# talmolab/track-mjx

Hardware: AMD Instinct MI355X
Metric: env-steps/sec (whole node), rodent task @ 4096 envs/GPU (higher is better)
Workload: dtype f32

## Files before the change

include/tmjx.h:

```cpp
#ifndef TMJX_H
#define TMJX_H
#include <stddef.h>
#include <stdint.h>

#ifdef __cplusplus
extern "C" {
#endif

#define TMJX_OK 0
#define TMJX_EINVAL (-22)
#define TMJX_ENOMEM (-12)
#define TMJX_EHIP (-5)

typedef struct tmjx_model tmjx_model;

typedef struct tmjx_layout_t {
  int32_t nq, nv, nu, nbody, ncon, nefc, obs_size, ref_obs_size, n_metrics, window;
  int32_t qpos, qvel, act, qacc_warmstart, time;
  int32_t xpos, xmat_torso, qfrc_actuator;
  int32_t prev_ctrl, action_buffer, done, steps_f;
  int32_t first_phys, first_obs, first_prev_ctrl;
  int32_t state_rows;
  int32_t i_clip_idx, i_start_frame, i_buffer_index, i_nan_count, istate_rows;
  int32_t ws_rows;
// ... 42 lines not shown
int tmjx_gae(const float *truncation, const float *termination, const float *rewards, const float *values,
             const float *bootstrap, float lambda_, float discount, float *vs, float *advantages, int T, int B,
             void *stream);

typedef struct {
  int32_t T, B, A, Z;
  float reward_scaling, discounting, gae_lambda, clip_eps, entropy_cost, kl_weight;
  int32_t normalize_advantage;
  int32_t accumulate;
} tmjx_ppo_cfg_t;
int tmjx_ppo_scratch_floats(int T, int B);
int tmjx_ppo_loss(const tmjx_ppo_cfg_t *cfg, const float *logits, const float *raw_action, const float *behaviour_logp,
                  const float *noise, const float *baseline, const float *bootstrap, const float *reward, const float *discount,
                  const float *truncation, const float *fc2, float *dlogits, float *dbaseline, float *dfc2, float *scratch,
                  float *out, void *stream);

#define TMJX_PPO_PHASE_A 1
#define TMJX_PPO_PHASE_B 2
#define TMJX_PPO_PHASE_C 4
#define TMJX_PPO_PHASE_D 8
int tmjx_ppo_loss_phases(const tmjx_ppo_cfg_t *cfg, const float *logits, const float *raw_action, const float *behaviour_logp,
                         const float *noise, const float *baseline, const float *bootstrap, const float *reward, const float *discount,
                         const float *truncation, const float *fc2, float *dlogits, float *dbaseline, float *dfc2, float *scratch,
                         float *out, int phases, void *stream);

int tmjx_silu_ln_partial_floats(int rows, int H);
int tmjx_silu_ln_fwd(const float *z, const float *bias, const float *gamma, const float *beta, float *y, float *stats, int rows, int H,
                     float eps, void *stream);
int tmjx_silu_ln_bwd(const float *dy, const float *z, const float *bias, const float *gamma, const float *stats, float *dz, float *grads,
                     float *partial, int rows, int H, void *stream);
int tmjx_silu_ln_fwd_bf16(const float *z, const float *bias, const float *gamma, const float *beta, uint16_t *y16, int ldy16, float *stats, int rows, int H,
                          float eps, void *stream);
int tmjx_silu_ln_bwd_bf16(const float *dy, const float *z, const float *bias, const float *gamma, const float *stats, uint16_t *dz16, int lddz16, float *grads,
                          float *partial, int rows, int H, void *stream);

int tmjx_gather_normalize(const float *src, const int64_t *idx, const float *mean, const float *std, float *out, int T, int R, int B,
                          int W, void *stream);
int tmjx_gather_minibatch(const float *obs, const float *next_last, const float *raw_action, const float *log_prob, const float *reward, const float *discount,
                          const float *truncation, const int64_t *idx, const float *mean, const float *std, float *obs_n, float *next_n, float *raw_action_g,
                          float *scalars_g, int T, int R, int B, int W, int A, void *stream);
#define TMJX_MINIBATCH_STATE_WORDS (16 + 16 * 64)
typedef struct tmjx_minibatch_t {
  const float *obs, *next_last, *raw_action, *log_prob, *reward, *discount, *truncation;
  const int64_t *perm;
  const float *mean, *std;
  float *obs_n, *next_n, *raw_action_g, *scalars_g;
  float *eps, *noise;
  int64_t *state;
  uint64_t seed;
  int32_t T, R, B, W, A, Z, advance;
} tmjx_minibatch_t;
int tmjx_minibatch_begin(const tmjx_minibatch_t *mb, void *stream);
int tmjx_minibatch_begin_bf16(const tmjx_minibatch_t *mb, uint16_t *obs_n16, int ld16, void *stream);
int tmjx_philox4x32_10(const uint32_t *ctr_key_dev, uint32_t *out_dev, void *stream);

int tmjx_latent_concat_bwd(const float *dx, const float *eps, const float *fc2, float *dfc2, int n, int Z, int dx_stride, void *stream);
int tmjx_latent_concat_bwd_add(const float *dx, const float *eps, const float *fc2, const float *add, float *dfc2, int n, int Z, int dx_stride,
                               void *stream);

int tmjx_latent_concat(const float *fc2, const float *eps, const float *obs, float *x, int n, int Z, int obs_w, int ref_w,
                       int64_t obs_s0, int64_t obs_s1, const float *mean, const float *std, int x_stride, uint64_t seed, const int64_t *rng_state,
                       void *stream);
int tmjx_sample_action(const float *logits, const float *noise, float *raw, float *action_t, float *logp, int n, int A, uint64_t seed,
                       int64_t *rng_state, void *stream);

int tmjx_linear_act_ok(const float *A, int64_t lda, const float *W, int ldw, int K);
int tmjx_linear_act(const float *A, int64_t lda, const float *W, int ldw, const float *bias, float *C, int M, int N, int K,
                    const float *mean, const float *inv_std, void *stream);
int tmjx_linear_nolds(const float *A, int64_t sa_row, int64_t sa_k, const float *W, const float *bias, float *C, int M, int N, int K,
                      void *stream);
int tmjx_linear_nolds_norm(const float *A, int64_t sa_row, int64_t sa_k, const float *W, const float *bias, float *C, int M, int N, int K,
                           const float *mean, const float *inv_std, void *stream);

int tmjx_linear_nolds_bf16(const float *A, int64_t sa_row, int64_t sa_k, const uint16_t *W, int ldw, const float *bias, float *C, int M, int N, int K,
                           const float *mean, const float *inv_std, void *stream);

int tmjx_colsum_scratch_floats(int width);
int tmjx_colsum(const float *src, float *out, float *scratch, int rows, int width, void *stream);

typedef struct tmjx_colsum_problem_t { const float *partial; float *out; int32_t rows, width; } tmjx_colsum_problem_t;
int tmjx_colsum_grouped(const tmjx_colsum_problem_t *problems, int n, void *stream);

int tmjx_adam_clip(float *param, const float *grad, float *exp_avg, float *exp_avg_sq, const float *grad_norm, long long n, float lr,
                   float beta1, float beta2, float eps, float bias_correction1, float bias_correction2, float max_norm, void *stream);
int tmjx_adam_norm_floats(void);
int tmjx_adam_clip_norm(float *param, const float *grad, float *exp_avg, float *exp_avg_sq, float *norm_scratch, float *norm_out, long long n, float lr,
                        float beta1, float beta2, float eps, float bias_correction1, float bias_correction2, float max_norm, void *stream);
int tmjx_adam_clip_norm_frozen(float *param, const float *grad, float *exp_avg, float *exp_avg_sq, float *norm_scratch, float *norm_out, long long n,
                               long long frozen_lo, long long frozen_hi, float lr, float beta1, float beta2, float eps, float bias_correction1,
                               float bias_correction2, float max_norm, void *stream);

int tmjx_gemm_nt(const float *A, int lda, const float *W, int ldw, const float *bias, float *C, int ldc, int M, int N, int K, void *stream);
int tmjx_gemm_nn(const float *A, int lda, const float *W, int ldw, float *C, int ldc, int M, int N, int K, void *stream);
int tmjx_gemm_nt_silu_ln_ok(const float *A, int lda, const float *W, int ldw, int N);
int tmjx_gemm_nt_silu_ln(const float *A, int lda, const float *W, int ldw, const float *bias, const float *gamma, const float *beta, float *Z, float *Y,
                         int ldc, float *stats, int M, int N, int K, float eps, void *stream);
int tmjx_gemm_nn_ln_bwd_ok(const float *dY, int ldy, const float *W, int ldw, int N);
long long tmjx_gemm_nn_ln_bwd_partial_floats(int M, int N);
int tmjx_gemm_nn_ln_bwd(const float *dY, int ldy, const float *W, int ldw, const float *z, const float *bias, const float *gamma, const float *stats,
                        float *dz, float *partial, int M, int N, int K, void *stream);
int tmjx_gemm_nt_silu_ok(const float *A, int lda, const float *W, int ldw);
int tmjx_gemm_nt_silu(const float *A, int lda, const float *W, int ldw, const float *bias, float *Z, float *Y, int ldc, int M, int N, int K, void *stream);
int tmjx_silu_fwd(const float *z, const float *bias, float *y, long long rows, int N, void *stream);
int tmjx_silu_bwd(const float *dy, const float *z, const float *bias, float *dz, long long rows, int N, void *stream);
int tmjx_gemm_nn_silu_bwd_ok(const float *dY, int ldy, const float *W, int ldw);
int tmjx_gemm_nn_silu_bwd(const float *dY, int ldy, const float *W, int ldw, const float *z, const float *bias, float *dZ, int M, int N, int K, void *stream);
int tmjx_silu_bwd_rank1(const float *dy1, const float *w1, const float *z, const float *bias, float *dz, long long rows, int N, void *stream);
long long tmjx_head_dw_scratch_floats(int M, int K);
int tmjx_head_dw(const float *dy1, const float *x, int ldx, float *dw, float *db, float *scratch, int M, int K, void *stream);
#define TMJX_CHAIN_MAX_HIDDEN 4
typedef struct { const float *W, *bias, *gamma, *beta; float *z, *y, *stats; int32_t K, ldw; } tmjx_chain_layer_t;
typedef struct {
  const float *A; int32_t lda, M, n_hidden, epi;
  tmjx_chain_layer_t hidden[TMJX_CHAIN_MAX_HIDDEN];
  const float *Wf, *bf; float *outf; int32_t Nf, ldwf, ldof;
  float eps;
  int32_t rows_alloc;
  void *prof;
} tmjx_chain_fwd_t;
int tmjx_chain_rows(int M);
int tmjx_chain_fwd_ok(const tmjx_chain_fwd_t *chain);
int tmjx_chain_fwd(const tmjx_chain_fwd_t *chain, void *stream);
typedef struct { const float *W; int32_t ldw; const float *z, *bias, *gamma, *stats; float *dz, *partial; } tmjx_chain_bwd_stage_t;
typedef struct {
  const float *G; int32_t ldg, Kg, M, n_stages, epi;
  tmjx_chain_bwd_stage_t stage[TMJX_CHAIN_MAX_HIDDEN];
  const float *W0; int32_t ldw0, dx_cols; float *dx; int32_t lddx;
  int32_t rows_alloc;
  void *prof;
} tmjx_chain_bwd_t;
int tmjx_chain_bwd_ok(const tmjx_chain_bwd_t *chain);
int tmjx_chain_bwd(const tmjx_chain_bwd_t *chain, void *stream);

int tmjx_head_fwd_ok(const float *x, int ldx, const float *w, int K);
int tmjx_head_fwd(const float *x, int ldx, const float *w, const float *bias, float *y, int M, int K, void *stream);
long long tmjx_gemm_dw_scratch_floats(int M, int N, int K);
int tmjx_gemm_dw(const float *dY, int ldy, const float *X, int ldx, float *dW, float *db, float *scratch, int M, int N, int K, void *stream);
typedef struct tmjx_dw_problem_t {
  const float *dY, *X;
  float *dW, *db, *scratch;
  int32_t ldy, ldx, lddw, M, N, K;
} tmjx_dw_problem_t;
int tmjx_gemm_dw_grouped(const tmjx_dw_problem_t *problems, int n, void *stream);

typedef struct tmjx_bf16_shadow_t {
  const float *src;
  uint16_t *dst, *dst_t;
  int32_t N, K, ld_src, ld_dst, ld_dst_t;
} tmjx_bf16_shadow_t;
int tmjx_bf16_shadow(const tmjx_bf16_shadow_t *items, int n, void *stream);
int tmjx_bgemm_nt(const void *A, int a_is_f32, int lda, const uint16_t *B, int ldb, const float *bias, float *C, int ldc, int M, int N, int K,
                  void *stream);
int tmjx_bgemm_row_tile_ok(int N);
int tmjx_bf16_z_bytes(void);
long long tmjx_bgemm_partial_floats(int M, int N, int sums);
int tmjx_bgemm_ln_fwd(const void *A, int a_is_f32, int lda, const uint16_t *B, int ldb, const float *bias, const float *gamma, const float *beta, uint16_t *Z16, int ldz,
                      uint16_t *Y16, int ldy16, float *stats, int M, int N, int K, float eps, void *stream);
int tmjx_bgemm_ln_bwd(const void *dY, int dy_is_f32, int ldy, const uint16_t *Bt, int ldb, const uint16_t *z16, int ldz, const float *bias, const float *gamma,
                      const float *stats, uint16_t *dZ16, int lddz, float *partial, int M, int N, int K, void *stream);
int tmjx_bgemm_silu_fwd(const void *A, int a_is_f32, int lda, const uint16_t *B, int ldb, const float *bias, uint16_t *Z16, int ldz, uint16_t *Y16, int ldy16,
                        float *Yf, int ldyf, int M, int N, int K, void *stream);
int tmjx_bgemm_silu_bwd(const void *dY, int dy_is_f32, int ldy, const uint16_t *Bt, int ldb, const uint16_t *z16, int ldz, const float *bias, uint16_t *dZ16, int lddz,
                        float *partial, int M, int N, int K, void *stream);
int tmjx_bf_silu_bwd(const float *dY, int ldy, const uint16_t *z16, int ldz, const float *bias, uint16_t *dZ16, int lddz, float *partial, int M, int N, void *stream);
int tmjx_bf_silu_bwd_rank1(const float *dy1, const float *w1, const uint16_t *z16, int ldz, const float *bias, uint16_t *dZ16, int lddz, float *partial, int M, int N,
                           void *stream);
long long tmjx_bgemm_dw_scratch_floats(int M, int N, int K);
int tmjx_bgemm_dw(const void *dY, int y_is_f32, int ldy, const void *X, int x_is_f32, int ldx, float *dW, int lddw, float *db, float *scratch,
                  int M, int N, int K, void *stream);
typedef struct tmjx_bdw_problem_t {
  const void *dY, *X;
  float *dW, *db, *scratch;
  int32_t y_is_f32, x_is_f32, ldy, ldx, lddw, M, N, K;
} tmjx_bdw_problem_t;
int tmjx_bgemm_dw_grouped(const tmjx_bdw_problem_t *problems, int n, int target_wgs, void *stream);

typedef struct tmjx_rollout_store_t {
  const float *obs; float *obs_dst0, *obs_dst1;
  const float *raw; float *raw_dst;
  const float *logp; float *logp_dst;
  const float *reward; float *reward_dst;
  const float *done; float *discount_dst;
  const float *trunc; float *trunc_dst;
  int32_t n, W, A;
  float *obs_dst2;
} tmjx_rollout_store_t;
int tmjx_rollout_store(const tmjx_rollout_store_t *s, void *stream);
int tmjx_clips_upload_velocities(tmjx_model *m, const float *velocity, const float *joints_velocity, int n_clips, int n_frames);
int tmjx_clips_share(tmjx_model *m, const tmjx_model *owner);

int tmjx_stats_scratch_floats(int W);
int tmjx_stats_sums(const float *src, const float *mean, float *sums, float *scratch, long long rows, int W, void *stream);
int tmjx_stats_apply(const float *sums, float n_added, float *count, float *mean, float *summed_variance, float *std, int W, float std_min,
                     float std_max, void *stream);
int tmjx_stats_apply_pinned(const float *sums, float n_added, float *count, float *mean, float *summed_variance, float *std, int W, int pin_lo,
                            float std_min, float std_max, void *stream);
// ... 299 lines not shown
```

track_mjx_amd/agent/losses.py:

```python
from __future__ import annotations

import ctypes as C

import torch

from .. import hip as _hip
from .networks import NormalTanh


def compute_gae(truncation, termination, rewards, values, bootstrap_value, lambda_: float = 1.0, discount: float = 0.99):
    T, B = rewards.shape
    args = [x.detach().contiguous().float() for x in (truncation, termination, rewards, values, bootstrap_value)]
    if not args[0].is_cuda:
        raise _hip.TmjxError("compute_gae runs on the GPU only (tmjx_gae); there is no CPU fallback")
    vs = torch.empty((T, B), dtype=torch.float32, device=rewards.device)
    adv = torch.empty_like(vs)
    L = _hip.lib()
    with torch.cuda.device(rewards.device):
        stream = C.c_void_p(torch.cuda.current_stream(rewards.device).cuda_stream)
        _hip.check(L.tmjx_gae(*[C.c_void_p(a.data_ptr()) for a in args], float(lambda_), float(discount),
                              C.c_void_p(vs.data_ptr()), C.c_void_p(adv.data_ptr()), T, B, stream), "tmjx_gae")
    return vs, adv


def gather_normalize(src: torch.Tensor, idx: torch.Tensor, normalizer) -> torch.Tensor:
    squeeze = src.dim() == 2
    if squeeze:
        src = src.unsqueeze(0)
    T, R, W = src.shape
    out = torch.empty((T, idx.shape[0], W), dtype=torch.float32, device=src.device)
    L = _hip.lib()
    with torch.cuda.device(src.device):
        stream = C.c_void_p(torch.cuda.current_stream(src.device).cuda_stream)
        _hip.check(L.tmjx_gather_normalize(*[C.c_void_p(t.data_ptr()) for t in (src, idx, normalizer.mean, normalizer.std, out)], T, R,
                                           idx.shape[0], W, stream), "tmjx_gather_normalize")
    return out[0] if squeeze else out


def gather_minibatch(buf: dict, idx: torch.Tensor, normalizer) -> dict:
    obs, nxt, act = buf["observation"], buf["next_observation_last"], buf["raw_action"]
    T, R, W = obs.shape
    B, A = idx.shape[0], act.shape[-1]
    f32 = dict(dtype=torch.float32, device=obs.device)
    obs_n, next_n = torch.empty((T, B, W), **f32), torch.empty((B, W), **f32)
    act_g, sc = torch.empty((T, B, A), **f32), torch.empty((4, T, B), **f32)
    p = lambda t: C.c_void_p(t.data_ptr())
    with torch.cuda.device(obs.device):
        _hip.check(_hip.lib().tmjx_gather_minibatch(p(obs), p(nxt), p(act), p(buf["log_prob"]), p(buf["reward"]), p(buf["discount"]), p(buf["truncation"]), p(idx),
                                                    p(normalizer.mean), p(normalizer.std), p(obs_n), p(next_n), p(act_g), p(sc), T, R, B, W, A,
                                                    C.c_void_p(torch.cuda.current_stream(obs.device).cuda_stream)), "tmjx_gather_minibatch")
    return {"observation_normalized": obs_n, "next_observation_last_normalized": next_n, "raw_action": act_g, "log_prob": sc[0], "reward": sc[1],
            "discount": sc[2], "truncation": sc[3]}


def minibatch_begin(buf: dict, perm: torch.Tensor, state: torch.Tensor, seed: int, normalizer, latents: int, advance: bool = True,
                    obs16: torch.Tensor | None = None) -> dict:
    obs, nxt, act = buf["observation"], buf["next_observation_last"], buf["raw_action"]
    T, R, W = obs.shape
    B, A = int(buf["_B"]), act.shape[-1]
    f32 = dict(dtype=torch.float32, device=obs.device)
    obs_n, next_n = torch.empty((T, B, W), **f32), torch.empty((B, W), **f32)
    act_g, sc = torch.empty((T, B, A), **f32), torch.empty((4, T, B), **f32)
    eps, noise = torch.empty((T, B, latents), **f32), torch.empty((T, B, A), **f32)
    d = lambda t: t.data_ptr()
    m = _hip.Minibatch(d(obs), d(nxt), d(act), d(buf["log_prob"]), d(buf["reward"]), d(buf["discount"]), d(buf["truncation"]), d(perm), d(normalizer.mean),
                       d(normalizer.std), d(obs_n), d(next_n), d(act_g), d(sc), d(eps), d(noise), d(state), seed & (2 ** 64 - 1), T, R, B, W, A, latents, int(advance))
    out = {"observation_normalized": obs_n, "next_observation_last_normalized": next_n, "raw_action": act_g, "log_prob": sc[0], "reward": sc[1],
           "discount": sc[2], "truncation": sc[3], "latent_eps": eps, "entropy_noise": noise}
    with torch.cuda.device(obs.device):
        stream = C.c_void_p(torch.cuda.current_stream(obs.device).cuda_stream)
        if obs16 is not None:
            assert obs16.dtype == torch.bfloat16 and obs16.shape[0] == T * B and obs16.shape[1] >= W and obs16.is_contiguous()
            _hip.check(_hip.lib().tmjx_minibatch_begin_bf16(C.byref(m), C.c_void_p(obs16.data_ptr()), obs16.shape[1], stream), "tmjx_minibatch_begin_bf16")
            out["observation_normalized_bf16"] = obs16
        else:
            _hip.check(_hip.lib().tmjx_minibatch_begin(C.byref(m), stream), "tmjx_minibatch_begin")
    return out


def create_ramp_schedule(max_value: float = 0.1, min_value: float = 0.0001, ramp_steps: int = 1000, warmup_steps: int = 0):
    def schedule_fn(step: float) -> float:
        if step < warmup_steps:
            return min_value
        progress = min(max((step - warmup_steps) / ramp_steps, min_value), 1.0)
        return progress * max_value
    return schedule_fn


class _FusedLossHead(torch.autograd.Function):

    @staticmethod
    def forward(ctx, logits, baseline, fc2, raw_action, behaviour_logp, noise, bootstrap, reward, discount, truncation, cfg):
        T, B = reward.shape
        dev = logits.device
        args = [a.detach().contiguous().float() for a in (logits, raw_action, behaviour_logp, noise, baseline, bootstrap, reward,
                                                          discount, truncation, fc2)]
        dlogits, dbaseline, dfc2 = torch.empty_like(args[0]), torch.empty_like(args[4]), torch.empty_like(args[9])
        L = _hip.lib()
        scratch = torch.empty(L.tmjx_ppo_scratch_floats(T, B), dtype=torch.float32, device=dev)
        out = torch.empty(8, dtype=torch.float32, device=dev)
        c = _hip.PpoCfg(T, B, raw_action.shape[-1], fc2.shape[-1] // 2, cfg["reward_scaling"], cfg["discounting"], cfg["gae_lambda"],
                        cfg["clipping_epsilon"], cfg["entropy_cost"], cfg["kl_weight"], int(cfg["normalize_advantage"]), 0)
        with torch.cuda.device(dev):
            stream = C.c_void_p(torch.cuda.current_stream(dev).cuda_stream)
            ptr = [C.c_void_p(a.data_ptr()) for a in args + [dlogits, dbaseline, dfc2, scratch, out]]
            _hip.check(L.tmjx_ppo_loss(C.byref(c), *ptr, stream), "tmjx_ppo_loss")
        ctx.save_for_backward(dlogits, dbaseline, dfc2)
        ctx.mark_non_differentiable(out)
        return out[0].clone(), out

    @staticmethod
    def backward(ctx, g_total, _g_out):
        dlogits, dbaseline, dfc2 = ctx.saved_tensors
        return (dlogits * g_total, dbaseline * g_total, dfc2 * g_total) + (None,) * 8


def ppo_loss_and_output_grads(policy, value, normalizer, data: dict, *, entropy_cost: float = 1e-4, kl_weight: float = 1e-3,
                              discounting: float = 0.9, reward_scaling: float = 1.0, gae_lambda: float = 0.95,
                              clipping_epsilon: float = 0.3, normalize_advantage: bool = True, side_stream=None, acc_out: torch.Tensor | None = None,
                              scalars_on_side: bool = False):
    obs = data["observation_normalized"] if "observation_normalized" in data else normalizer.normalize(data["observation"])
    nxt = data["next_observation_last_normalized"] if "next_observation_last_normalized" in data else normalizer.normalize(data["next_observation_last"])
    T, B = data["reward"].shape
    dev = obs.device
    L = _hip.lib()
    phased = side_stream is not None and T <= 24
    cfg_of = lambda A_, Z_: _hip.PpoCfg(T, B, A_, Z_, reward_scaling, discounting, gae_lambda, clipping_epsilon, entropy_cost, kl_weight,
                                        int(normalize_advantage), int(acc_out is not None))
    f32 = lambda a: a.detach().contiguous().float()
    if side_stream is not None:
        cur = torch.cuda.current_stream(dev)
        with torch.no_grad():
            scratch = torch.empty(L.tmjx_ppo_scratch_floats(T, B), dtype=torch.float32, device=dev)
            out = torch.empty(8, dtype=torch.float32, device=dev) if acc_out is None else acc_out
            row = [f32(data[k]) for k in ("raw_action", "log_prob", "reward", "discount", "truncation")]
        side_stream.wait_stream(cur)
        with torch.cuda.stream(side_stream):
            with torch.no_grad():
                bootstrap = value(nxt)
            baseline = value(obs)
            if phased:
                with torch.no_grad():
                    bl, bs = f32(baseline), f32(bootstrap)
        logits, fc2 = policy(obs, eps=data.get("latent_eps"), return_fc2=True)
        if not phased:
            cur.wait_stream(side_stream)
        baseline.record_stream(cur); bootstrap.record_stream(cur)
    else:
        logits, fc2 = policy(obs, eps=data.get("latent_eps"), return_fc2=True)
        baseline = value(obs)
        with torch.no_grad():
            bootstrap = value(nxt)
    with torch.no_grad():
        noise = data["entropy_noise"] if "entropy_noise" in data else torch.randn(data["raw_action"].shape, dtype=torch.float32, device=logits.device)
        if phased:
            lg, nz, f2 = f32(logits), f32(noise), f32(fc2)
            dlogits, dbaseline, dfc2 = torch.empty_like(lg), torch.empty_like(bl), torch.empty_like(f2)
            c = cfg_of(data["raw_action"].shape[-1], fc2.shape[-1] // 2)
            args = [lg, row[0], row[1], nz, bl, bs, row[2], row[3], row[4], f2]
            ptr = [C.c_void_p(a.data_ptr()) for a in args + [dlogits, dbaseline, dfc2, scratch, out]]
            for t_ in (scratch, out, dbaseline, *row):
                t_.record_stream(side_stream)
            for t_ in (bl, bs):
                t_.record_stream(cur)

            def phase(mask, stream):
                _hip.check(L.tmjx_ppo_loss_phases(C.byref(c), *ptr, mask, C.c_void_p(stream.cuda_stream)), "tmjx_ppo_loss_phases")
            with torch.cuda.device(dev):
                phase(2, side_stream)
                cur.wait_stream(side_stream)
                phase(1 | 4, cur)
                if scalars_on_side:
                    side_stream.wait_stream(cur)
                    phase(8, side_stream)
                else:
                    phase(8, cur)
            args9 = f2
        else:
            args = [f32(a) for a in (logits, data["raw_action"], data["log_prob"], noise, baseline, bootstrap, data["reward"],
                                     data["discount"], data["truncation"], fc2)]
            dlogits, dbaseline, dfc2 = torch.empty_like(args[0]), torch.empty_like(args[4]), torch.empty_like(args[9])
            if side_stream is None:
                scratch = torch.empty(L.tmjx_ppo_scratch_floats(T, B), dtype=torch.float32, device=dev)
                out = torch.empty(8, dtype=torch.float32, device=dev) if acc_out is None else acc_out
            c = cfg_of(data["raw_action"].shape[-1], fc2.shape[-1] // 2)
            with torch.cuda.device(dev):
                stream = C.c_void_p(torch.cuda.current_stream(dev).cuda_stream)
                ptr = [C.c_void_p(a.data_ptr()) for a in args + [dlogits, dbaseline, dfc2, scratch, out]]
                _hip.check(L.tmjx_ppo_loss(C.byref(c), *ptr, stream), "tmjx_ppo_loss")
            args9 = args[9]
    metrics = {"total_loss": out[0], "policy_loss": out[1], "v_loss": out[2], "kl_latent_loss": out[4], "entropy_loss": out[3]}
    handle = getattr(policy, "latent_grad_handle", None)
    if handle is not None and handle.matches(fc2) and args9.data_ptr() == fc2.data_ptr():
        handle.add(dfc2.view(-1, fc2.shape[-1]))
        return metrics, (logits, baseline), (dlogits.view_as(logits), dbaseline.view_as(baseline)), out
    return metrics, (logits, baseline, fc2), (dlogits.view_as(logits), dbaseline.view_as(baseline), dfc2.view_as(fc2)), out


def compute_ppo_loss_fused(policy, value, normalizer, data: dict, *, entropy_cost: float = 1e-4, kl_weight: float = 1e-3,
                           discounting: float = 0.9, reward_scaling: float = 1.0, gae_lambda: float = 0.95,
                           clipping_epsilon: float = 0.3, normalize_advantage: bool = True):
    obs = data["observation_normalized"] if "observation_normalized" in data else normalizer.normalize(data["observation"])
# ... 54 lines not shown
```

track_mjx_amd/agent/networks.py:

```python
from __future__ import annotations

import math
import os
from typing import Sequence

import torch
import torch.nn as nn
import torch.nn.functional as F


def _lecun_uniform_(w: torch.Tensor) -> None:
    fan_in = w.shape[1]
    lim = math.sqrt(3.0 / fan_in)
    with torch.no_grad():
        w.uniform_(-lim, lim)


def _lecun_normal_(w: torch.Tensor) -> None:
    fan_in = w.shape[1]
    std = math.sqrt(1.0 / fan_in) / 0.87962566103423978
    with torch.no_grad():
        nn.init.trunc_normal_(w, mean=0.0, std=std, a=-2 * std, b=2 * std)


# ... 172 lines not shown
    return dz[:, :N], partial.view(-1, N)


class Bf16Shadows:

    def __init__(self, linears, need_t=None):
        from .. import hip as _hip
        self.lins = list(linears)
        need_t = set(self.lins if need_t is None else need_t)
        dev = self.lins[0].weight.device
        self.w, self.wt = {}, {}
        items = []
        for lin in self.lins:
            N, K = lin.weight.shape
            self.w[lin] = torch.zeros((N, _ceil64(K)), dtype=torch.bfloat16, device=dev)
            if lin in need_t:
                self.wt[lin] = torch.zeros((K, _ceil64(N)), dtype=torch.bfloat16, device=dev)
            t = self.wt.get(lin)
            items.append(_hip.Bf16Shadow(lin.weight.data_ptr(), self.w[lin].data_ptr(), t.data_ptr() if t is not None else None, N, K, lin.weight.stride(0),
                                         self.w[lin].stride(0), t.stride(0) if t is not None else 0))
        self._chunks = [(_hip.Bf16Shadow * len(items[i:i + 24]))(*items[i:i + 24]) for i in range(0, len(items), 24)]
        self._ptrs = [lin.weight.data_ptr() for lin in self.lins]

    def refresh(self) -> None:
        if self._ptrs != [lin.weight.data_ptr() for lin in self.lins]:
            raise RuntimeError("a parameter moved after its bf16 shadow was built (build the shadows after the flat optimiser re-seats the parameters)")
        dev = self.lins[0].weight.device
        for arr in self._chunks:
            _launch("tmjx_bf16_shadow", dev, arr, len(arr))


def _bf16_ok(x, lin) -> bool:
    sh = gemm_inputs.shadows
    return (gemm_inputs.dtype == torch.bfloat16 and sh is not None and lin in sh.w and x.is_cuda and x.dtype == torch.float32
            and lin.out_features % 4 == 0)


def _colsum(dy: torch.Tensor) -> torch.Tensor:
    if not (dy.is_cuda and dy.dtype == torch.float32 and dy.dim() == 2 and dy.is_contiguous() and dy.shape[0] >= 1024):
        return dy.sum(0)
    from .. import hip as _hip
    rows, width = dy.shape
    out = torch.empty(width, dtype=torch.float32, device=dy.device)
    scratch = torch.empty(_hip.lib().tmjx_colsum_scratch_floats(width), dtype=torch.float32, device=dy.device)
    _launch("tmjx_colsum", dy.device, _p(dy), _p(out), _p(scratch), rows, width)
    return out


class deferred_weight_grads:
    active = None

    def __enter__(self):
        self.problems, self.keep, self.colsums = [], [], []
        self.bproblems = []
        self.seen: set = set()
        deferred_weight_grads.active = self
        return self

    def __exit__(self, *a):
        deferred_weight_grads.active = None
        return False

    @staticmethod
    def _aligned(t):
        return t.data_ptr() % 16 == 0 and t.stride(0) % 4 == 0 and t.stride(1) == 1

    def try_add(self, dy2, x2, w, b):
        gw, gb = w.grad, (b.grad if b is not None else None)
        if gw is None or (b is not None and gb is None) or len(self.problems) >= 16:
            return None
        if not (self._aligned(dy2) and self._aligned(x2) and gw.stride(1) == 1 and gw.shape == w.shape):
            return None
        if id(w) in self.seen:
            mine = [q for q in self.problems if q[2].data_ptr() == gw.data_ptr()]
            self.problems = [q for q in self.problems if q[2].data_ptr() != gw.data_ptr()]
            self._launch_problems(mine)
            return None
        self.seen.add(id(w))
        self.problems.append((dy2, x2, gw, gb))
        return gw, gb

    def launch(self):
        from .. import hip as _hip
        if self.colsums:
            dev = self.colsums[0][0].device
            arr = (_hip.ColsumProblem * len(self.colsums))(*[_hip.ColsumProblem(pt.data_ptr(), g.data_ptr(), nb, wd) for pt, g, nb, wd in self.colsums])
            _launch("tmjx_colsum_grouped", dev, arr, len(self.colsums))
            self.keep += [t for c in self.colsums for t in c[:2]]
            self.colsums = []
        self._launch_problems(self.problems)
        self.problems = []
        self._launch_bproblems()

    def _launch_bproblems(self):
        from .. import hip as _hip
        probs, self.bproblems = self.bproblems, []
        if not probs:
            return
        L = _hip.lib()
        dev = probs[0][0].device
        for at in range(0, len(probs), 24):
            grp = probs[at:at + 24]
            sizes = [int(L.tmjx_bgemm_dw_scratch_floats(dy.shape[0], dy.shape[1], x.shape[1])) for dy, x, _, _ in grp]
            scratch = torch.empty(sum((n + 3) // 4 * 4 for n in sizes), dtype=torch.float32, device=dev)
            arr = (_hip.BdwProblem * len(grp))()
            off = 0
            for i, (dy, x, dw, db) in enumerate(grp):
                N, K = dy.shape[1], x.shape[1]
                arr[i] = _hip.BdwProblem(dy.data_ptr(), x.data_ptr(), dw.data_ptr(), db.data_ptr() if db is not None else None, scratch.data_ptr() + 4 * off,
                                         int(dy.dtype == torch.float32), int(x.dtype == torch.float32), _ld(dy), _ld(x), dw.stride(0) if N > 1 else max(dw.stride(0), K),
                                         dy.shape[0], N, K)
                off += (sizes[i] + 3) // 4 * 4
            _launch("tmjx_bgemm_dw_grouped", dev, arr, len(grp), 0)
            self.keep += [scratch] + [t for q in grp for t in q[:2]]

    def _launch_problems(self, problems):
        from .. import hip as _hip
        if not problems:
            return
        L = _hip.lib()
        dev = problems[0][0].device
        sizes = [int(L.tmjx_gemm_dw_scratch_floats(dy.shape[0], dy.shape[1], x.shape[1])) for dy, x, _, _ in problems]
        scratch = torch.empty(sum((n + 3) // 4 * 4 for n in sizes), dtype=torch.float32, device=dev)
        arr = (_hip.DwProblem * len(problems))()
        off = 0
        for i, (dy, x, gw, gb) in enumerate(problems):
            arr[i] = _hip.DwProblem(dy.data_ptr(), x.data_ptr(), gw.data_ptr(), gb.data_ptr() if gb is not None else None,
                                    scratch.data_ptr() + 4 * off, dy.stride(0), x.stride(0), gw.stride(0), dy.shape[0], dy.shape[1], x.shape[1])
            off += (sizes[i] + 3) // 4 * 4
        _launch("tmjx_gemm_dw_grouped", dev, arr, len(problems))
        self.keep += [scratch] + [t for q in problems for t in q[:2]]


def chain_fwd_desc(x2, hidden, final=None, kind="ln", eps=1e-6, out=None):
    from .. import hip as _hip
    M, dev = x2.shape[0], x2.device
    d = _hip.ChainFwd()
    d.A, d.lda, d.M, d.n_hidden, d.epi, d.eps = x2.data_ptr(), x2.stride(0), M, len(hidden), 1 if kind == "ln" else 3, float(eps)
    saved = []
    d.rows_alloc = rows = int(_hip.lib().tmjx_chain_rows(M))
    for l, h in enumerate(hidden):
        w, b = h[0], h[1]
        z = torch.empty((M, 256), dtype=torch.float32, device=dev)
        y = torch.empty((rows, 256), dtype=torch.float32, device=dev)[:M]
        st = torch.empty((M, 2), dtype=torch.float32, device=dev) if kind == "ln" else None
        L = d.hidden[l]
        L.W, L.bias, L.z, L.y, L.K, L.ldw = w.data_ptr(), b.data_ptr(), z.data_ptr(), y.data_ptr(), w.shape[1], w.stride(0)
        if kind == "ln":
            L.gamma, L.beta, L.stats = h[2].data_ptr(), h[3].data_ptr(), st.data_ptr()
        saved.append((z, y, st))
    if final is not None:
        wf, bf = final
        Nf = wf.shape[0]
        if out is None:
            out = torch.empty((M,) if Nf == 1 else (M, Nf), dtype=torch.float32, device=dev)
        d.Wf, d.bf, d.outf, d.Nf, d.ldwf, d.ldof = wf.data_ptr(), (bf.data_ptr() if bf is not None else None), out.data_ptr(), Nf, wf.stride(0), (1 if Nf == 1 else out.stride(0))
    return d, saved, out


def chain_fwd(x2, hidden, final=None, kind="ln", eps=1e-6):
    import ctypes as C
    d, saved, out = chain_fwd_desc(x2, hidden, final, kind, eps)
    _launch("tmjx_chain_fwd", x2.device, C.byref(d))
    return saved, out


def chain_fwd_ok(x2, hidden, final=None, kind="ln") -> bool:
    import ctypes as C
    from .. import hip as _hip
    if os.environ.get("TMJX_NO_CHAIN") or not (x2.is_cuda and x2.dtype == torch.float32 and x2.dim() == 2 and x2.stride(1) == 1):
        return False
    if any(h[0].shape[0] != 256 for h in hidden) or not (1 <= len(hidden) <= 4):
        return False
    return bool(_hip.lib().tmjx_chain_fwd_ok(C.byref(chain_fwd_desc(x2[:1], hidden, final, kind)[0])))


def chain_bwd(g, final_w, blocks, kind="ln", w0=None, dx_cols=None, prof=None, dx_ld=None):
    import ctypes as C
    from .. import hip as _hip
    L = _hip.lib()
    M, dev = g.shape[0], g.device
    d = _hip.ChainBwd()
    head = g.dim() == 1
# ... 182 lines not shown
        for L in layers:
            out += [grads.get(id(p)) for p in L.params()]
        return (dx, None, None, None, None, *out)


def bf16_chain(x, layers, dx_cols=None, last_y_f32=False):
    params = [p for L in layers for p in L.params()]
    return _BfChainFn.apply(x, layers, gemm_inputs.shadows, dx_cols, last_y_f32, *params)


def _bf16_chain_ok(x) -> bool:
    sh = gemm_inputs.shadows
    return gemm_inputs.dtype == torch.bfloat16 and sh is not None and x.is_cuda and x.dtype in (torch.float32, torch.bfloat16)



class _F32ChainFn(torch.autograd.Function):

    @staticmethod
    def forward(ctx, x, layers, dx_cols, *params):
        x2 = _rows2d(x)
        hid, last = layers[:-1], layers[-1]
        kind = hid[0].kind
        hidden = [(L.lin.weight, L.lin.bias, L.norm.weight, L.norm.bias) if kind == "ln" else (L.lin.weight, L.lin.bias) for L in hid]
        eps = float(hid[0].norm.eps) if kind == "ln" else 0.0
        saved, out = chain_fwd(x2, hidden, (last.lin.weight, last.lin.bias), kind, eps)
        flat = [t for z, y, st in saved for t in ((z, y, st) if kind == "ln" else (z, y))]
        ctx.save_for_backward(x2, *flat, *params)
        ctx.layers, ctx.dx_cols, ctx.x_shape, ctx.kind, ctx.nflat = layers, dx_cols, x.shape, kind, len(flat)
        return out.view(*x.shape[:-1], last.lin.out_features) if last.kind == "dense" else out.view(*x.shape[:-1], 1)

    @staticmethod
    def backward(ctx, dout):
        from .. import hip as _hip
        layers, kind = ctx.layers, ctx.kind
        hid, last = layers[:-1], layers[-1]
        st_ = ctx.saved_tensors
        x2, flat, params = st_[0], st_[1:1 + ctx.nflat], st_[1 + ctx.nflat:]
        per = 3 if kind == "ln" else 2
        saved = [flat[per * i:per * i + per] for i in range(len(hid))]
        pit = iter(params)
        P = [[next(pit) for _ in L.params()] for L in layers]
        Lh = _hip.lib()
        dev = dout.device
        M = x2.shape[0]
        d = deferred_weight_grads.active
        grads: dict = {}
        wf, bf = P[-1][0], P[-1][1]
        y_last = saved[-1][1]
        if last.kind == "head":
            g = dout.reshape(-1)
            g = g if g.is_contiguous() else g.contiguous()
            K = wf.shape[1]
            dwh, dbh = torch.empty((1, K), dtype=torch.float32, device=dev), torch.empty(1, dtype=torch.float32, device=dev)
            scratch = torch.empty(int(Lh.tmjx_head_dw_scratch_floats(M, K)), dtype=torch.float32, device=dev)
            _launch("tmjx_head_dw", dev, _p(g), _p(y_last), y_last.stride(0), _p(dwh), _p(dbh), _p(scratch), M, K)
            grads[(len(layers) - 1, 0)], grads[(len(layers) - 1, 1)] = dwh, dbh
            ctx._keep = scratch
        else:
            g = _rows2d(dout)
            if g.data_ptr() % 16 or g.stride(0) % 4:
                g = g.contiguous()
            got = d.try_add(g, y_last, last.lin.weight, last.lin.bias) if d is not None else None
            dw, db = got if got is not None else gemm_dw(g, y_last, True)
            grads[(len(layers) - 1, 0)], grads[(len(layers) - 1, 1)] = dw, db
        if kind == "ln":
            blocks = [(P[l][0], saved[l][0], P[l][1], P[l][2], saved[l][2]) for l in range(len(hid) - 1, -1, -1)]
        else:
            blocks = [(P[l][0], saved[l][0], P[l][1]) for l in range(len(hid) - 1, -1, -1)]
        want_dx = ctx.needs_input_grad[0]
        cols = (x2.shape[1] if ctx.dx_cols is None else int(ctx.dx_cols)) if want_dx else None
        dzs, partials, dx = chain_bwd(g, wf, blocks, kind, P[0][0] if want_dx else None, cols, dx_ld=x2.shape[1] if want_dx else None)
        for i, dz in enumerate(dzs):
            l = len(hid) - 1 - i
            L = hid[l]
            xin = x2 if l == 0 else saved[l - 1][1]
            if kind == "ln":
                got = d.try_add(dz, xin, L.lin.weight, None) if d is not None else None
                grads[(l, 0)] = got[0] if got is not None else gemm_dw(dz, xin, False)[0]
                g3 = torch.empty((3, 256), dtype=torch.float32, device=dev)
                nblk = partials[i].numel() // 768
                if d is not None and len(d.colsums) < 16:
                    d.colsums.append((partials[i], g3, nblk, 768))
                else:
                    one = (_hip.ColsumProblem * 1)(_hip.ColsumProblem(partials[i].data_ptr(), g3.data_ptr(), nblk, 768))
                    _launch("tmjx_colsum_grouped", dev, one, 1)
                grads[(l, 2)], grads[(l, 3)], grads[(l, 1)] = g3[0], g3[1], g3[2]
            else:
                got = d.try_add(dz, xin, L.lin.weight, L.lin.bias) if d is not None else None
                grads[(l, 0)], grads[(l, 1)] = got if got is not None else gemm_dw(dz, xin, True)
        out = [grads.get((l, j)) for l, L in enumerate(layers) for j in range(len(L.params()))]
        return (dx.view(ctx.x_shape) if dx is not None else None, None, None, *out)


def f32_chain(x, layers, dx_cols=None):
    params = [p for L in layers for p in L.params()]
    return _F32ChainFn.apply(x, layers, dx_cols, *params)


def _f32_chain_ok(x, layers, dx_cols=None) -> bool:
    if gemm_inputs.dtype is not None or torch.is_autocast_enabled() or os.environ.get("TMJX_NO_CHAIN") or not (x.is_cuda and x.dtype == torch.float32):
        return False
    if x.requires_grad and torch.is_grad_enabled() and (x.shape[-1] if dx_cols is None else int(dx_cols)) > 128:
        return False
    hid, last = layers[:-1], layers[-1]
    if not hid or any(L.lin.out_features != 256 or L.lin.bias is None for L in hid) or last.lin.bias is None or last.lin.in_features != 256:
        return False
    kind = hid[0].kind
    hidden = [(L.lin.weight, L.lin.bias, L.norm.weight, L.norm.bias) if kind == "ln" else (L.lin.weight, L.lin.bias) for L in hid]
    return chain_fwd_ok(_rows2d(x), hidden, (last.lin.weight, last.lin.bias), kind)


class _BlockLink:
    __slots__ = ("y_ptr", "y_shape", "ctx", "dz_given", "grads")

    def __init__(self):
        self.y_ptr, self.y_shape, self.ctx, self.dz_given, self.grads = None, None, None, False, None


class ln_bwd_links:
    active = False
    last = None

    def __enter__(self):
        self._prev = (ln_bwd_links.active, ln_bwd_links.last)
        ln_bwd_links.active, ln_bwd_links.last = not os.environ.get("TMJX_NO_LN_BWD_FUSION"), None
        return self

    def __exit__(self, *a):
        ln_bwd_links.active, ln_bwd_links.last = self._prev
        return False

    @staticmethod
    def producer_of(x2):
# ... 310 lines not shown
        d = deferred_weight_grads.active
        got = d.try_add(dz, x2, ctx.param, None) if d is not None else None
        dw = got[0] if got is not None else gemm_dw(dz, x2, False)[0]
        return dx, dw, grads[2], grads[0], grads[1], None, None


class _Block(nn.Module):
    FUSED_WIDTHS = (64, 128, 256, 512, 1024)

    def __init__(self, i: int, o: int):
        super().__init__()
        self.dense = _dense(i, o)
        self.norm = nn.LayerNorm(o, eps=1e-6)
        self.dx_cols = None

    def forward(self, x):
        if x.is_cuda and x.dtype == torch.float32 and self.dense.out_features in self.FUSED_WIDTHS and not torch.is_autocast_enabled():
            x2 = _rows2d(x)
            if torch.is_grad_enabled() and _block_fusable(x2, self.dense.weight):
                y = _HipBlockFn.apply(x2, self.dense.weight, self.dense.bias, self.norm.weight, self.norm.bias, self.norm.eps, self.dx_cols)
                return y.view(*x.shape[:-1], self.dense.out_features)
            if _bf16_ok(x2, self.dense):
                if torch.is_grad_enabled():
                    z = _BfDenseFn.apply(x2, self.dense.weight, None, self.dense, self.dx_cols)
                else:
                    z = bgemm_nt(x2, gemm_inputs.shadows.w[self.dense], self.dense.out_features, self.dense.in_features)
            elif not torch.is_grad_enabled():
                z = gemm_nt(x2, self.dense.weight)
            else:
                z = _HipDenseFn.apply(x2, self.dense.weight, None, self.dx_cols)
            y = _SiluLayerNormFn.apply(z, self.dense.bias, self.norm.weight, self.norm.bias, self.norm.eps)
            return y.view(*x.shape[:-1], self.dense.out_features)
        return self.norm(F.silu(self.dense(x)))


class _LatentConcatFn(torch.autograd.Function):

    @staticmethod
    def forward(ctx, fc2, eps, obs, ref, handle=None):
        ctx.handle = handle
        n, Z = eps.shape
        W = obs.shape[1]
        fc2, eps, obs = fc2.contiguous(), eps.contiguous(), obs.contiguous()
        wd = Z + W - ref
        x = torch.empty((n, (wd + 3) // 4 * 4), dtype=torch.float32, device=fc2.device)
        _launch("tmjx_latent_concat", fc2.device, _p(fc2), _p(eps), _p(obs), _p(x), n, Z, W, ref, obs.stride(0), obs.stride(1), None, None, x.shape[1], 0, None)
        ctx.save_for_backward(fc2, eps)
        return x[:, :wd]

    @staticmethod
    def backward(ctx, dx):
        fc2, eps = ctx.saved_tensors
        n, Z = eps.shape
        dx = dx.contiguous()
        dfc2 = torch.empty_like(fc2)
        add = ctx.handle.take() if ctx.handle is not None else None
        if add is not None and (add.shape != fc2.shape or not add.is_contiguous()):
            raise RuntimeError("_LatentConcatFn: the pending fc2 gradient does not fit this forward pass")
        if add is None:
            _launch("tmjx_latent_concat_bwd", fc2.device, _p(dx), _p(eps), _p(fc2), _p(dfc2), n, Z, dx.shape[1])
        else:
            _launch("tmjx_latent_concat_bwd_add", fc2.device, _p(dx), _p(eps), _p(fc2), _p(add), _p(dfc2), n, Z, dx.shape[1])
        return dfc2, None, None, None, None


class LatentGradHandle:

    def __init__(self, fc2: torch.Tensor):
        self.ptr, self.shape, self._g = fc2.data_ptr(), tuple(fc2.shape), None

    def matches(self, fc2: torch.Tensor) -> bool:
        return fc2.data_ptr() == self.ptr

    def add(self, g: torch.Tensor) -> None:
        if self._g is not None:
            raise RuntimeError("LatentGradHandle: a gradient is already parked on this forward pass")
        self._g = g

    def take(self):
        g, self._g = self._g, None
        return g

    @property
    def pending(self) -> bool:
        return self._g is not None


class IntentionPolicy(nn.Module):

    def __init__(self, obs_size: int, reference_obs_size: int, action_size: int, latents: int = 60,
                 encoder_layers: Sequence[int] = (1024, 1024), decoder_layers: Sequence[int] = (1024, 1024)):
        super().__init__()
        self.reference_obs_size, self.latents, self.action_size = reference_obs_size, latents, action_size
        enc, d = [], reference_obs_size
        for h in encoder_layers:
            enc.append(_Block(d, h)); d = h
        self.encoder = nn.Sequential(*enc)
        self.fc2 = _dense(d, 2 * latents, _lecun_normal_)
        dec, d = [], latents + (obs_size - reference_obs_size)
        for h in decoder_layers:
            dec.append(_Block(d, h)); d = h
        self.decoder = nn.Sequential(*dec)
        dec[0].dx_cols = latents
        self.head = _dense(d, 2 * action_size)

    def forward(self, obs: torch.Tensor, eps: torch.Tensor | None = None, deterministic: bool = False, return_fc2: bool = False):
        traj = obs[..., :self.reference_obs_size]
        prev, self.latent_grad_handle = getattr(self, "latent_grad_handle", None), None
        if prev is not None and prev.pending:
            raise RuntimeError("IntentionPolicy: the fc2 gradient parked on the previous forward pass (LatentGradHandle.add) was never consumed by a "
                               "backward pass through that forward — it would have been dropped")
        chains = _bf16_chain_ok(obs) and all(m.out_features % 4 == 0 for m in (self.fc2, self.head))
        if chains:
            if getattr(self, "_enc_chain", None) is None:
                self._enc_chain = [_Layer("ln", b.dense, b.norm) for b in self.encoder] + [_Layer("dense", self.fc2)]
                self._dec_chain = [_Layer("ln", b.dense, b.norm) for b in self.decoder] + [_Layer("dense", self.head)]
            fc2 = bf16_chain(traj, self._enc_chain)
        else:
            if getattr(self, "_enc_f32", None) is None and obs.is_cuda:
                self._enc_f32 = [_Layer("ln", b.dense, b.norm) for b in self.encoder] + [_Layer("dense", self.fc2)]
                self._dec_f32 = [_Layer("ln", b.dense, b.norm) for b in self.decoder] + [_Layer("dense", self.head)]
            if obs.is_cuda and _f32_chain_ok(traj, self._enc_f32):
                fc2 = f32_chain(traj, self._enc_f32)
            else:
                with ln_bwd_links():
                    h = self.encoder(traj)
                    fc2 = self.fc2(h)
        mean, logvar = torch.chunk(fc2, 2, dim=-1)
        if (not deterministic and fc2.is_cuda and fc2.dtype == torch.float32 and obs.dtype == torch.float32 and not torch.is_autocast_enabled()
                and fc2.numel() >= 2 * self.latents * 1024):
            lead = fc2.shape[:-1]
            if eps is None:
                eps = torch.randn_like(mean)
            handle = LatentGradHandle(fc2.reshape(-1, fc2.shape[-1])) if (fc2.requires_grad and fc2.is_contiguous()) else None
            x = _LatentConcatFn.apply(fc2.reshape(-1, fc2.shape[-1]), eps.reshape(-1, self.latents), obs.reshape(-1, obs.shape[-1]), self.reference_obs_size, handle)
            self.latent_grad_handle = handle
            x = x.view(*lead, x.shape[-1])
            if chains:
                logits = bf16_chain(x, self._dec_chain, dx_cols=self.latents)
            elif _f32_chain_ok(x, self._dec_f32, self.latents):
                logits = f32_chain(x, self._dec_f32, dx_cols=self.latents)
            else:
                with ln_bwd_links():
                    logits = self.head(self.decoder(x))
            if return_fc2:
                return logits, fc2
            return logits, mean, logvar
        if deterministic:
            z = mean
        else:
            if eps is None:
                eps = torch.randn_like(mean)
            z = mean + eps * torch.exp(0.5 * logvar)
        x = torch.cat([z, obs[..., self.reference_obs_size:]], dim=-1)
        logits = bf16_chain(x, self._dec_chain) if chains else self.head(self.decoder(x))
        if return_fc2:
            return logits, fc2
        return logits, mean, logvar


class DecoderNet(nn.Module):

    def __init__(self, input_size: int, action_size: int, decoder_layers: Sequence[int] = (1024, 1024)):
        super().__init__()
        self.action_size = action_size
        dec, d = [], input_size
        for h in decoder_layers:
            dec.append(_Block(d, h)); d = h
        self.decoder = nn.Sequential(*dec)
        self.head = _dense(d, 2 * action_size)

    def forward(self, x: torch.Tensor) -> torch.Tensor:
        return self.head(self.decoder(x))


class _NoCtx:
    def save_for_backward(self, *a):
        pass


class ValueNet(nn.Module):

    def __init__(self, obs_size: int, hidden: Sequence[int] = (1024, 1024)):
        super().__init__()
        layers, d = [], obs_size
        for h in hidden:
            layers += [_dense(d, h), nn.SiLU()]; d = h
        layers.append(_dense(d, 1))
# ... 139 lines not shown
```

track_mjx_amd/agent/ppo.py:

```python
from __future__ import annotations

import logging
import math
import time
from typing import Callable

import numpy as np
import torch
import torch.distributed as dist

from . import losses as _losses
from .networks import Bf16Shadows, IntentionPolicy, NormalTanh, RunningStatistics, ValueNet, deferred_weight_grads, gemm_inputs


import contextlib
import gc
import os


@contextlib.contextmanager
def _capture(graph):
    gc.collect()
    enabled = gc.isenabled()
    gc.disable()
# ... 559 lines not shown
        offs = [0]
        for e in self.envs:
            offs.append(offs[-1] + e.num_envs)
        self._refresh_padded_weights()
        cur = torch.cuda.current_stream(self.dev) if self._streams else None
        if self._streams:
            for sg in self._streams:
                sg.wait_stream(cur)
        jax_noise = self.sgd_keys is not None and self.act_rng == "jax"
        if jax_noise:
            self.sgd_keys.start_unrolls()
        for u in range(self.unrolls):
            if jax_noise:
                self.sgd_keys.start_unroll()
            for t in range(T):
                if jax_noise:
                    eps_np, noise_np = self.sgd_keys.act_noise(n_local, self.policy.latents, self.policy.action_size)
                    eps_all, noise_all = torch.from_numpy(eps_np).to(self.dev), torch.from_numpy(noise_np).to(self.dev)
                    if self._streams:
                        ev = torch.cuda.Event()
                        ev.record(torch.cuda.current_stream(self.dev))
                        for sg in self._streams:
                            sg.wait_event(ev)
                            eps_all.record_stream(sg); noise_all.record_stream(sg)
                for g, env in enumerate(self.envs):
                    sl = slice(u * n_local + offs[g], u * n_local + offs[g + 1])
                    with torch.cuda.stream(self._streams[g]) if self._streams else _nullctx():
                        st = self.states[g]
                        if u == 0 and t == 0:
                            self.buf["observation"][0, sl] = st.obs
                            if self._obs_rm is not None:
                                self._obs_rm[g].copy_(st.obs)
                        if jax_noise:
                            action, extra = self.act(st.obs, draws=(eps_all[offs[g]:offs[g + 1]], noise_all[offs[g]:offs[g + 1]]))
                        else:
                            action, extra = self._act_graphed(st.obs if self._obs_rm is None else self._obs_rm[g], g)
                        st = env.step(st, action)
                        nxt = self.buf["observation"][t + 1, sl] if t + 1 < T else self.buf["next_observation_last"][sl]
                        nxt1 = self.buf["observation"][0, slice(sl.start + n_local, sl.stop + n_local)] if (t + 1 == T and u + 1 < self.unrolls) else None
                        self._store_transition(env, st, extra, nxt, nxt1, t, sl, None if self._obs_rm is None else self._obs_rm[g])
                        self.states[g] = st
        if self._streams:
            for sg in self._streams:
                cur.wait_stream(sg)

    def _self_advancing(self) -> bool:
        return (self.dev.type == "cuda" and self.normalize_observations and self.buf["observation"].shape[-1] % 4 == 0
                and all(v.is_contiguous() for v in self.buf.values()))

    def _mb_data(self, idx):
        fused_gather = self.dev.type == "cuda" and self.normalize_observations and self.buf["observation"].shape[-1] % 4 == 0
        if idx is None:
            data = _losses.minibatch_begin({**self.buf, "_B": self.local_batch}, self._perm_static, self._mb_state, self._noise_seed, self.normalizer,
                                           self.policy.latents, obs16=self._obs16)
        elif fused_gather and all(v.is_contiguous() for v in self.buf.values()):
            data = _losses.gather_minibatch(self.buf, idx, self.normalizer)
        else:
            data = {k: (self.buf[k].index_select(1, idx) if k != "next_observation_last" else self.buf[k].index_select(0, idx)) for k in self.buf}
        if self.shadows is not None:
            self.shadows.refresh()
        return data

    def _mb_forward(self, idx, kl_w, scalars_on_side: bool = False):
        data = self._mb_data(idx)
        twins = None
        if "observation_normalized_bf16" in data:
            on = data["observation_normalized"]
            twins = {on.data_ptr(): (data["observation_normalized_bf16"], on.shape[-1])}
        with gemm_inputs(self.matmul_dtype, self.shadows, twins):
            m, outs, gouts, out8 = _losses.ppo_loss_and_output_grads(self.policy, self.value, self.normalizer, data, kl_weight=kl_w,
                                                                     side_stream=self._sgd_side, acc_out=self._acc8 if idx is None else None,
                                                                     scalars_on_side=scalars_on_side and self._sgd_side is not None, **self.hp)
        return outs, gouts, out8

    def _mb_backward(self, outs, gouts, which: str = "all"):
        npol = self._n_policy_params
        if which == "all":
            o, g, params = list(outs), list(gouts), self.grads.params
        elif which == "value":
            o, g, params = [outs[1]], [gouts[1]], self.grads.params[npol:]
        else:
            o, g, params = [outs[0]] + list(outs[2:]), [gouts[0]] + list(gouts[2:]), self.grads.params[:npol]
        with gemm_inputs(self.matmul_dtype, self.shadows):
            with deferred_weight_grads() as dwg:
                grads = torch.autograd.grad(o, params, grad_outputs=g)
            if which != "policy" and self._sgd_side is not None:
                torch.cuda.current_stream(self.dev).wait_stream(self._sgd_side)
            dwg.launch()
        setattr(self, "_dwg_" + which, dwg)
        if which == "all":
            self.grads.assign(grads)
        else:
            self.grads.assign_subset(params, grads)

    def _minibatch_grads(self, idx: torch.Tensor | None, kl_w: float) -> torch.Tensor:
        if self.dev.type == "cuda":
            outs, gouts, out8 = self._mb_forward(idx, kl_w, scalars_on_side=True)
            self._mb_backward(outs, gouts, "all")
            if idx is None:
                return self._acc8
            return out8[self._metric_index]
        data = self._mb_data(idx)
        with gemm_inputs(self.matmul_dtype, self.shadows):
            loss, m = _losses.compute_ppo_loss(self.policy, self.value, self.normalizer, data, kl_weight=kl_w, **self.hp,
                                               **({"gae_fn": self.gae_fn} if self.gae_fn is not None else {}))
        self.grads.assign(torch.autograd.grad(loss, self.grads.params))
        return torch.stack([m[k].float() for k in self.METRIC_KEYS])
# ... 359 lines not shown
```

track_mjx_amd/csrc/gemm_kernels.h:

```cpp
#pragma once
#include "silu_math.h"
#include <type_traits>

typedef float __attribute__((ext_vector_type(4))) gf4;
typedef float __attribute__((ext_vector_type(2))) gf2;

#define GEMM_BM 80
#define GEMM_BK 32
#define GEMM_A_ROWS (GEMM_BM + 8)
#define GEMM_LDA 40

template <bool VEC>
__device__ __forceinline__ gf4 gemm_ld4(const float *__restrict__ p, long long row_off, int k, int K, bool row_ok, int &mask) {
  const float *q = p + (row_ok ? row_off : 0ll);
  const bool any = row_ok && k < K;
  const int left = any ? K - k : 0;
  mask = left >= 4 ? 15 : (1 << (left > 0 ? left : 0)) - 1;
  gf4 v;
  if (VEC) {
    v = *reinterpret_cast<const gf4 *>(q + (any ? k : 0));
  } else {
    const int last = K - 1;
    v.x = q[any ? k : 0];
    v.y = q[any ? min(k + 1, last) : 0];
// ... 638 lines not shown
        if (col + 1 < K) *reinterpret_cast<gf2 *>(o) = gf2{acc[a][0][r], acc[a][1][r]};
        else if (col < K) o[0] = acc[a][0][r];
      }
    }
}
template <bool YVEC, bool XVEC>
__global__ __launch_bounds__(512) void k_gemm_dw(const float *__restrict__ dY, int ldy, const float *__restrict__ X, int ldx, float *__restrict__ slabs,
                                                 int M, int N, int K, int with_bias, int rows_per_split, int ld_slab) {
  gemm_dw_tile<YVEC, XVEC>(dY, ldy, X, ldx, slabs, M, N, K, with_bias, rows_per_split, ld_slab, blockIdx.x, blockIdx.y, blockIdx.z);
}
__device__ __forceinline__ void dw_reduce_elem(const float *__restrict__ slabs, float *__restrict__ dW, float *__restrict__ db, int S, int N, int K,
                                               int with_bias, int ld_slab, int lddw, long long i) {
  const int Kx = K + (with_bias ? 1 : 0);
  if (i >= (long long)N * Kx) return;
  const int n = (int)(i / Kx), k = (int)(i % Kx);
  const float *p = slabs + (size_t)n * ld_slab + k;
  const size_t step = (size_t)N * ld_slab;
  float a[8] = {0.f, 0.f, 0.f, 0.f, 0.f, 0.f, 0.f, 0.f};
  int s = 0;
  for (; s + 8 <= S; s += 8) {
#pragma unroll
    for (int u = 0; u < 8; u++) a[u] += p[(size_t)(s + u) * step];
  }
  for (; s < S; s++) a[0] += p[(size_t)s * step];
  const float v = ((a[0] + a[1]) + (a[2] + a[3])) + ((a[4] + a[5]) + (a[6] + a[7]));
  if (k < K) dW[(size_t)n * lddw + k] = v; else db[n] = v;
}
__global__ __launch_bounds__(256) void k_dw_reduce(const float *__restrict__ slabs, float *__restrict__ dW, float *__restrict__ db, int S, int N, int K,
                                                   int with_bias, int ld_slab, int lddw) {
  dw_reduce_elem(slabs, dW, db, S, N, K, with_bias, ld_slab, lddw, (long long)blockIdx.x * 256 + threadIdx.x);
}

#define DW_GROUP_MAX 16
struct DwProblem {
  const float *dY, *X;
  float *dW, *db, *slabs;
  int ldy, ldx, lddw, M, N, K, rows_per_split, S, ld_slab, tiles_n, tiles_k;
  int wg_begin, red_begin;
};
struct DwGroup { DwProblem p[DW_GROUP_MAX]; int n; };
__global__ __launch_bounds__(512) void k_gemm_dw_grouped(const DwGroup G) {
  int i = 0;
  for (int j = 1; j < G.n; j++) if ((int)blockIdx.x >= G.p[j].wg_begin) i = j;
  const DwProblem &P = G.p[i];
  const int local = blockIdx.x - P.wg_begin, tiles = P.tiles_n * P.tiles_k, split = local / tiles, tl = local % tiles;
  gemm_dw_tile<true, true>(P.dY, P.ldy, P.X, P.ldx, P.slabs, P.M, P.N, P.K, P.db != nullptr, P.rows_per_split, P.ld_slab, tl / P.tiles_k, tl % P.tiles_k, split);
}
__global__ __launch_bounds__(256) void k_dw_reduce_grouped(const DwGroup G) {
  int i = 0;
  for (int j = 1; j < G.n; j++) if ((int)blockIdx.x >= G.p[j].red_begin) i = j;
  const DwProblem &P = G.p[i];
  dw_reduce_elem(P.slabs, P.dW, P.db, P.S, P.N, P.K, P.db != nullptr, P.ld_slab, P.lddw, (long long)(blockIdx.x - P.red_begin) * 256 + threadIdx.x);
}
#endif
```

track_mjx_amd/csrc/ppo_kernels.h:

```cpp
#pragma once
#include "silu_math.h"
#include "act_shared.h"
#include <hip/hip_runtime.h>
#include <math.h>

struct PpoCfg {
  int T, B, A, Z;
  float reward_scaling, discounting, gae_lambda, clip_eps, entropy_cost, kl_weight;
  int normalize_advantage;
  int accumulate;
};

#define PPO_BLOCK 256
#define PPO_ALPHA 0.95f
__device__ __forceinline__ float ppo_sigmoid(float x) { return 1.f / (1.f + expf(-x)); }

template <int NV>
__device__ __forceinline__ void ppo_block_sum(float *v, float *lds) {
  const int tid = threadIdx.x, lane = tid & 63, w = tid >> 6, nw = (blockDim.x + 63) >> 6;
#pragma unroll
  for (int k = 0; k < NV; k++) {
    float x = v[k];
    for (int off = 32; off >= 1; off >>= 1) x += __shfl_xor(x, off);
    if (lane == 0) lds[k * 16 + w] = x;
// ... 610 lines not shown
#pragma unroll
      for (int b = 0; b < NB; b++) fw[b] = *reinterpret_cast<const f4 *>(sW + (wc + 16 * b + li) * ACT_LD + 16 * c + 4 * kq);
#pragma unroll
      for (int e = 0; e < 4; e++)
#pragma unroll
        for (int a = 0; a < 2; a++)
#pragma unroll
          for (int b = 0; b < NB; b++) acc[a][b] = __builtin_amdgcn_mfma_f32_16x16x4f32(fa[a][e], fw[b][e], acc[a][b], 0, 0, 0);
    }
  }
#pragma unroll
  for (int a = 0; a < 2; a++)
#pragma unroll
    for (int b = 0; b < NB; b++) {
      const int c = col0 + wc + 16 * b + li;
      const float bv = (bias && c < N) ? bias[c] : 0.f;
#pragma unroll
      for (int r = 0; r < 4; r++) {
        const int row = row0 + wr + 16 * a + 4 * kq + r;
        if (row < M && c < N) C[(size_t)row * N + c] = acc[a][b][r] + bv;
      }
    }
}

__global__ __launch_bounds__(256) void k_gather_normalize(const float *__restrict__ src, const long long *__restrict__ idx, const float *__restrict__ mean,
                                                          const float *__restrict__ stdv, float *__restrict__ out, int T, int R, int B, int W) {
  const int w4 = W >> 2;
  const size_t total = (size_t)T * B * w4;
  for (size_t i = (size_t)blockIdx.x * 256 + threadIdx.x; i < total; i += (size_t)gridDim.x * 256) {
    int c = (int)(i % w4);
    size_t tb = i / w4;
    int b = (int)(tb % B), t = (int)(tb / B);
    const float4 v = reinterpret_cast<const float4 *>(src + ((size_t)t * R + (size_t)idx[b]) * W)[c];
    const float4 m = reinterpret_cast<const float4 *>(mean)[c], s = reinterpret_cast<const float4 *>(stdv)[c];
    float4 o = {(v.x - m.x) / s.x, (v.y - m.y) / s.y, (v.z - m.z) / s.z, (v.w - m.w) / s.w};
    reinterpret_cast<float4 *>(out + tb * W)[c] = o;
  }
}

#define TM_MB_SUBTICKETS 64
#define TM_MB_STATE_HEAD 16
#define TM_MB_STATE_STRIDE 16
struct MinibatchGather {
  const float *obs, *next_last, *raw_action, *scalar[4];
  const long long *idx;
  const float *mean, *stdv;
  float *obs_n, *next_n, *raw_action_g, *scalars_g;
  float *eps, *noise;
  long long *state;
  unsigned long long seed;
  int T, R, B, W, A, Z, advance;
  unsigned short *obs_n16; int ld16;
};
__global__ __launch_bounds__(256) void k_gather_minibatch(MinibatchGather g) {
  const int w4 = g.W >> 2;
  const unsigned long long ctr = g.state ? (unsigned long long)g.state[0] : 0ull;
  const long long *idx = g.idx + (g.state ? g.state[1] * (long long)g.B : 0ll);
  const size_t n_obs = (size_t)g.T * g.B * w4, n_next = (size_t)g.B * w4, n_act = (size_t)g.T * g.B * g.A, n_sc = (size_t)4 * g.T * g.B;
  const size_t q_eps = g.eps ? ((size_t)g.T * g.B * g.Z + 3) / 4 : 0, q_noise = g.noise ? (n_act + 3) / 4 : 0;
  const size_t e0 = n_obs + n_next, e1 = e0 + n_act, e2 = e1 + n_sc, e3 = e2 + q_eps, total = e3 + q_noise;
  for (size_t i = (size_t)blockIdx.x * 256 + threadIdx.x; i < total; i += (size_t)gridDim.x * 256) {
    if (i < e0) {
      const bool nx = i >= n_obs;
      const size_t j = nx ? i - n_obs : i;
      const int c = (int)(j % w4);
      const size_t tb = j / w4;
      const int b = (int)(tb % g.B), t = (int)(tb / g.B);
      const float *src = nx ? g.next_last : g.obs;
      const float4 v = reinterpret_cast<const float4 *>(src + ((size_t)t * g.R + (size_t)idx[b]) * g.W)[c];
      const float4 m = reinterpret_cast<const float4 *>(g.mean)[c], s = reinterpret_cast<const float4 *>(g.stdv)[c];
      const float4 o = {(v.x - m.x) / s.x, (v.y - m.y) / s.y, (v.z - m.z) / s.z, (v.w - m.w) / s.w};
      reinterpret_cast<float4 *>((nx ? g.next_n : g.obs_n) + tb * g.W)[c] = o;
      if (!nx && g.obs_n16) *reinterpret_cast<uint2 *>(g.obs_n16 + tb * g.ld16 + 4 * c) = uint2{silu_ln_pack(o.x, o.y), silu_ln_pack(o.z, o.w)};
    } else if (i < e1) {
      const size_t j = i - e0;
      const int c = (int)(j % g.A);
      const size_t tb = j / g.A;
      const int b = (int)(tb % g.B), t = (int)(tb / g.B);
      g.raw_action_g[j] = g.raw_action[((size_t)t * g.R + (size_t)idx[b]) * g.A + c];
    } else if (i < e2) {
      const size_t j = i - e1;
      const int b = (int)(j % g.B);
      const size_t kt = j / g.B;
      const int t = (int)(kt % g.T), k = (int)(kt / g.T);
      g.scalars_g[j] = g.scalar[k][(size_t)t * g.R + (size_t)idx[b]];
    } else {
      const bool second = i >= e3;
      const size_t q = second ? i - e3 : i - e2, n = second ? n_act : (size_t)g.T * g.B * g.Z;
      float v[4];
      tm_normal4(g.seed, ctr, second ? 1u : 0u, (unsigned)q, v);
      float *dst = second ? g.noise : g.eps;
#pragma unroll
      for (int k = 0; k < 4; k++) if (4 * q + k < n) dst[4 * q + k] = v[k];
    }
  }
  if (g.state && g.advance) {
    __syncthreads();
    if (threadIdx.x == 0) {
      const unsigned sub = blockIdx.x % TM_MB_SUBTICKETS, nsub = min((unsigned)gridDim.x, (unsigned)TM_MB_SUBTICKETS);
      const unsigned members = (gridDim.x - sub + TM_MB_SUBTICKETS - 1) / TM_MB_SUBTICKETS;
      unsigned long long *st = (unsigned long long *)g.state, *subt = st + TM_MB_STATE_HEAD + (size_t)TM_MB_STATE_STRIDE * sub;
      if (__hip_atomic_fetch_add(subt, 1ull, __ATOMIC_RELAXED, __HIP_MEMORY_SCOPE_AGENT) == (unsigned long long)members - 1ull) {
        __hip_atomic_store(subt, 0ull, __ATOMIC_RELAXED, __HIP_MEMORY_SCOPE_AGENT);
        if (__hip_atomic_fetch_add(st + 2, 1ull, __ATOMIC_RELAXED, __HIP_MEMORY_SCOPE_AGENT) == (unsigned long long)nsub - 1ull) {
          __hip_atomic_store(st + 2, 0ull, __ATOMIC_RELAXED, __HIP_MEMORY_SCOPE_AGENT);
          g.state[0] += 1; g.state[1] += 1;
        }
      }
    }
  }
}
__global__ void k_philox_kat(const unsigned *ctr_key, unsigned *out) {
  if (threadIdx.x == 0) tm_philox4x32_10(ctr_key[0], ctr_key[1], ctr_key[2], ctr_key[3], ctr_key[4], ctr_key[5], out);
}

__global__ __launch_bounds__(256) void k_latent_concat(const float *__restrict__ fc2, const float *__restrict__ eps, const float *__restrict__ obs,
                                                       float *__restrict__ x, int n, int Z, int obs_w, int ref_w, long long obs_s0, long long obs_s1,
                                                       const float *__restrict__ mean, const float *__restrict__ stdv, int x_stride,
                                                       unsigned long long seed, const long long *__restrict__ rng_state) {
  TM_PRIO_ACTING();
  const int W = Z + obs_w - ref_w;
  const unsigned long long ctr = rng_state ? (unsigned long long)rng_state[0] : 0ull;
  for (size_t i = (size_t)blockIdx.x * blockDim.x + threadIdx.x; i < (size_t)n * x_stride; i += (size_t)gridDim.x * blockDim.x) {
    int c = (int)(i % x_stride); size_t e = i / x_stride;
    float v = 0.f;
    if (c < Z) {
      v = tm_latent_sample(tm_normal_at(eps, seed, ctr, 2u, e * Z + c), fc2[e * 2 * Z + Z + c], fc2[e * 2 * Z + c]);
    } else if (c < W) { int k = ref_w + c - Z; v = obs[(long long)e * obs_s0 + (long long)k * obs_s1]; if (mean) v = tm_obs_normalised(v, mean[k], stdv[k]); }
    x[e * (size_t)x_stride + c] = v;
  }
}
__global__ __launch_bounds__(256) void k_latent_concat_bwd(const float *__restrict__ dx, const float *__restrict__ eps, const float *__restrict__ fc2,
                                                           float *__restrict__ dfc2, int n, int Z, int dx_stride, const float *__restrict__ add) {
  for (size_t i = (size_t)blockIdx.x * 256 + threadIdx.x; i < (size_t)n * Z; i += (size_t)gridDim.x * 256) {
    int c = (int)(i % Z); size_t e = i / Z;
    float g = dx[e * (size_t)dx_stride + c];
    float gm = g, gv = g * eps[e * Z + c] * (0.5f * expf(0.5f * fc2[e * 2 * Z + Z + c]));
    if (add) { gm = add[e * 2 * Z + c] + gm; gv = add[e * 2 * Z + Z + c] + gv; }
    dfc2[e * 2 * Z + c] = gm;
    dfc2[e * 2 * Z + Z + c] = gv;
  }
}
__global__ __launch_bounds__(PPO_BLOCK) void k_sample_action(const float *__restrict__ logits, const float *__restrict__ noise, float *__restrict__ raw,
                                                             float *__restrict__ action_t, float *__restrict__ logp, int n, int A,
                                                             unsigned long long seed, long long *__restrict__ rng_state) {
  TM_PRIO_ACTING();
  const int gid = blockIdx.x * blockDim.x + threadIdx.x, e = gid / PPO_G, sub = gid % PPO_G;
  const unsigned long long ctr = rng_state ? (unsigned long long)rng_state[0] : 0ull;
  float lp = 0.f;
  if (e < n) lp = sample_action_lane(logits + (size_t)e * 2 * A, noise, raw, action_t, n, A, (size_t)e, sub, seed, ctr);
  lp = ppo_group_sum(lp);
  if (e < n && sub == 0) logp[e] = lp;
  if (rng_state) {
    __syncthreads();
    if (threadIdx.x == 0) {
      unsigned long long *st = (unsigned long long *)rng_state;
      if (__hip_atomic_fetch_add(st + 1, 1ull, __ATOMIC_RELAXED, __HIP_MEMORY_SCOPE_AGENT) == (unsigned long long)gridDim.x - 1ull) {
        __hip_atomic_store(st + 1, 0ull, __ATOMIC_RELAXED, __HIP_MEMORY_SCOPE_AGENT);
        rng_state[0] += 1;
      }
    }
  }
}

#define NL_TM 4
#define NL_TN 4
template <int V> struct NlVec;
template <> struct NlVec<4> { typedef float4 T; };
template <> struct NlVec<2> { typedef float2 T; };
template <> struct NlVec<1> { typedef float T; };
template <int V> __device__ __forceinline__ void nl_unpack(const typename NlVec<V>::T &v, float *o);
template <> __device__ __forceinline__ void nl_unpack<4>(const float4 &v, float *o) { o[0] = v.x; o[1] = v.y; o[2] = v.z; o[3] = v.w; }
template <> __device__ __forceinline__ void nl_unpack<2>(const float2 &v, float *o) { o[0] = v.x; o[1] = v.y; }
template <> __device__ __forceinline__ void nl_unpack<1>(const float &v, float *o) { o[0] = v; }

template <int V, bool A_KMAJOR>
__global__ __launch_bounds__(128) void k_linear_nolds(const float *__restrict__ A, long long sa_row, long long sa_k, const float *__restrict__ W,
                                                      const float *__restrict__ bias, float *__restrict__ C, int M, int N, int K) {
  TM_PRIO_ACTING();
  typedef typename NlVec<V>::T VT;
  const int tx = threadIdx.x & 7, ty = threadIdx.x >> 3;
  const int row0 = blockIdx.x * 64 + ty * NL_TM, col0 = blockIdx.y * 32 + tx * NL_TN;
  float acc[NL_TM][NL_TN];
#pragma unroll
  for (int i = 0; i < NL_TM; i++)
#pragma unroll
    for (int j = 0; j < NL_TN; j++) acc[i][j] = 0.f;
  int cc[NL_TN];
#pragma unroll
  for (int j = 0; j < NL_TN; j++) cc[j] = col0 + j < N ? col0 + j : N - 1;
  const int rbase = row0 + NL_TM <= M ? row0 : (M >= NL_TM ? M - NL_TM : 0);
  int rr[NL_TM];
#pragma unroll
// ... 80 lines not shown
  const float scale = max_norm / fmaxf(max_norm, nrm);
  const float step = lr / bc1, rs = 1.f / sqrtf(bc2);
  for (long long i = (long long)blockIdx.x * 256 + threadIdx.x; i < n; i += (long long)gridDim.x * 256) {
    float gi = g[i] * scale;
    float mi = b1 * m[i] + (1.f - b1) * gi;
    float vi = b2 * v[i] + (1.f - b2) * gi * gi;
    m[i] = mi; v[i] = vi;
    p[i] -= step * mi / (sqrtf(vi) * rs + eps);
  }
}
__global__ __launch_bounds__(256) void k_adam_clip_frozen(float *__restrict__ p, const float *__restrict__ g, float *__restrict__ m, float *__restrict__ v,
                                                          const float *__restrict__ grad_norm, long long n, long long lo, long long hi, float lr, float b1,
                                                          float b2, float eps, float bc1, float bc2, float max_norm, float *__restrict__ norm_out) {
  __shared__ float lds[4];
  float s = wave_sum(grad_norm[threadIdx.x]);
  if ((threadIdx.x & 63) == 0) lds[threadIdx.x >> 6] = s;
  __syncthreads();
  const float nrm = sqrtf((lds[0] + lds[1]) + (lds[2] + lds[3]));
  if (norm_out && blockIdx.x == 0 && threadIdx.x == 0) norm_out[0] = nrm;
  const float scale = max_norm / fmaxf(max_norm, nrm);
  const float step = lr / bc1, rs = 1.f / sqrtf(bc2);
  for (long long i = (long long)blockIdx.x * 256 + threadIdx.x; i < n; i += (long long)gridDim.x * 256) {
    float gi = g[i] * scale;
    float mi = b1 * m[i] + (1.f - b1) * gi;
    float vi = b2 * v[i] + (1.f - b2) * gi * gi;
    m[i] = mi; v[i] = vi;
    if (i < lo || i >= hi) p[i] -= step * mi / (sqrtf(vi) * rs + eps);
  }
}

#define COLSUM_CHUNKS 64
__global__ __launch_bounds__(256) void k_colsum_rows(const float *__restrict__ src, float *__restrict__ partial, int rows, int width) {
  __shared__ float lds[8][33];
  const int cx = threadIdx.x & 31, ry = threadIdx.x >> 5, col = blockIdx.x * 32 + cx;
  const int per = (rows + COLSUM_CHUNKS - 1) / COLSUM_CHUNKS, r0 = blockIdx.y * per, r1 = r0 + per < rows ? r0 + per : rows;
  float acc[8] = {0.f, 0.f, 0.f, 0.f, 0.f, 0.f, 0.f, 0.f};
  if (col < width) {
    int r = r0 + ry;
    for (; r + 56 < r1; r += 64) {
#pragma unroll
      for (int u = 0; u < 8; u++) acc[u] += src[(size_t)(r + 8 * u) * width + col];
    }
    for (; r < r1; r += 8) acc[0] += src[(size_t)r * width + col];
  }
  lds[ry][cx] = ((acc[0] + acc[1]) + (acc[2] + acc[3])) + ((acc[4] + acc[5]) + (acc[6] + acc[7]));
  __syncthreads();
  if (ry == 0 && col < width) { float s = 0.f; for (int j = 0; j < 8; j++) s += lds[j][cx]; partial[(size_t)blockIdx.y * width + col] = s; }
}


#define COLSUM_GROUP_MAX 16
struct ColsumProblem { const float *partial; float *out; int nblk, width, blk_begin; };
struct ColsumGroup { ColsumProblem p[COLSUM_GROUP_MAX]; int n; };
__global__ __launch_bounds__(256) void k_colsum_grouped(const ColsumGroup G) {
  __shared__ float lds[8][33];
  int i = 0;
  for (int j = 1; j < G.n; j++) if ((int)blockIdx.x >= G.p[j].blk_begin) i = j;
  const ColsumProblem &P = G.p[i];
  const int cx = threadIdx.x & 31, ry = threadIdx.x >> 5, col = (blockIdx.x - P.blk_begin) * 32 + cx;
  float acc[8] = {0.f, 0.f, 0.f, 0.f, 0.f, 0.f, 0.f, 0.f};
  if (col < P.width) {
    int k = ry;
    for (; k + 56 < P.nblk; k += 64) {
#pragma unroll
      for (int u = 0; u < 8; u++) acc[u] += P.partial[(size_t)(k + 8 * u) * P.width + col];
    }
    for (; k < P.nblk; k += 8) acc[0] += P.partial[(size_t)k * P.width + col];
  }
  lds[ry][cx] = ((acc[0] + acc[1]) + (acc[2] + acc[3])) + ((acc[4] + acc[5]) + (acc[6] + acc[7]));
  __syncthreads();
  if (ry == 0 && col < P.width) { float s = 0.f; for (int j = 0; j < 8; j++) s += lds[j][cx]; P.out[col] = s; }
}

#define STATS_SLABS 512
__global__ __launch_bounds__(256) void k_stats_partial(const float *__restrict__ src, const float *__restrict__ mean, float *__restrict__ partial,
                                                       long long rows, int W) {
  typedef float __attribute__((ext_vector_type(4))) f4;
  __shared__ f4 lds[2][4][64];
  const int cx = threadIdx.x & 63, ry = threadIdx.x >> 6, c4 = blockIdx.x * 64 + cx, W4 = W >> 2;
  const long long per = (rows + STATS_SLABS - 1) / STATS_SLABS, r0 = blockIdx.y * per, r1 = r0 + per < rows ? r0 + per : rows;
  f4 s1 = {0.f, 0.f, 0.f, 0.f}, s2 = {0.f, 0.f, 0.f, 0.f};
  if (c4 < W4) {
    const f4 m = ((const f4 *)mean)[c4];
    const f4 *p = (const f4 *)src + c4;
    long long r = r0 + ry;
    for (; r + 28 < r1; r += 32) {
      f4 v[8];
#pragma unroll
      for (int u = 0; u < 8; u++) v[u] = p[(size_t)(r + 4 * u) * W4];
#pragma unroll
      for (int u = 0; u < 8; u++) { f4 d = v[u] - m; s1 += d; s2 += d * d; }
    }
    for (; r < r1; r += 4) { f4 d = p[(size_t)r * W4] - m; s1 += d; s2 += d * d; }
  }
  lds[0][ry][cx] = s1; lds[1][ry][cx] = s2;
  __syncthreads();
  if (ry == 0 && c4 < W4) {
    f4 a = (lds[0][0][cx] + lds[0][1][cx]) + (lds[0][2][cx] + lds[0][3][cx]), b = (lds[1][0][cx] + lds[1][1][cx]) + (lds[1][2][cx] + lds[1][3][cx]);
    ((f4 *)(partial + (size_t)blockIdx.y * 2 * W))[c4] = a;
    ((f4 *)(partial + (size_t)blockIdx.y * 2 * W + W))[c4] = b;
  }
}
__global__ void k_stats_finalize(const float *__restrict__ sums, float n_added, float *count, float *mean, float *summed_variance, float *std,
                                 int W, float std_min, float std_max) {
  const int c = blockIdx.x * blockDim.x + threadIdx.x;
  const float cnt = *count + n_added;
  if (c < W) {
    const float s1 = sums[c], s2 = sums[W + c];
    const float upd = s1 / cnt;
    const float sv = summed_variance[c] + (s2 - upd * s1);
    mean[c] += upd;
    summed_variance[c] = sv;
    std[c] = fminf(fmaxf(sqrtf(fmaxf(sv, 0.f) / cnt), std_min), std_max);
  }
}
__global__ void k_stats_count(float *count, float n_added) { *count += n_added; }
__global__ void k_stats_finalize_pinned(const float *__restrict__ sums, float n_added, float *count, float *mean, float *summed_variance, float *std,
                                        int W, int pin_lo, float std_min, float std_max) {
  const int c = blockIdx.x * blockDim.x + threadIdx.x;
  const float cnt = *count + n_added;
  if (c < pin_lo) {
    const float s1 = sums[c], s2 = sums[W + c];
    const float upd = s1 / cnt;
    const float sv = summed_variance[c] + (s2 - upd * s1);
    mean[c] += upd;
// ... 141 lines not shown
```

track_mjx_amd/csrc/tmjx_hip.hip:

```cpp
#include <hip/hip_runtime.h>

#include <stdlib.h>

#include <string>
#include <vector>

#include "../../include/tmjx.h"
#include "env_core.h"
#include "host_launch.h"
#include "model_host.h"
#include "wave_physics.h"
#ifdef TMJX_LANE_IMPL
#include "../../tests/lane/physics_core.h"
#endif

struct tmjx_model {
  DModel h;
  DModel *d = nullptr;
  float *clips[7] = {nullptr, nullptr, nullptr, nullptr, nullptr, nullptr, nullptr};
  int block = 64;
  int wave = 1;
  bool rodent = false;
  mutable float *mspill = nullptr;
  mutable int mspill_envs = 0;
// ... 707 lines not shown
  switch (H) { case 64: TMJX_FWD(1); break; case 128: TMJX_FWD(2); break; case 256: TMJX_FWD(4); break; case 512: TMJX_FWD(8); break;
               case 1024: TMJX_FWD(16); break; default: return fail(TMJX_EINVAL, "H must be 64, 128, 256, 512 or 1024"); }
#undef TMJX_FWD
  return check_launch("k_silu_ln_fwd");
}
int tmjx_silu_ln_fwd(const float *z, const float *bias, const float *gamma, const float *beta, float *y, float *stats, int rows, int H,
                     float eps, void *stream) {
  if (!y) return fail(TMJX_EINVAL, "null argument");
  return silu_ln_fwd_any(z, bias, gamma, beta, y, nullptr, 0, stats, rows, H, eps, stream);
}
int tmjx_silu_ln_fwd_bf16(const float *z, const float *bias, const float *gamma, const float *beta, uint16_t *y16, int ldy16, float *stats, int rows, int H,
                          float eps, void *stream) {
  if (!y16) return fail(TMJX_EINVAL, "null argument");
  return silu_ln_fwd_any(z, bias, gamma, beta, nullptr, y16, ldy16, stats, rows, H, eps, stream);
}

static int silu_ln_bwd_any(const float *dy, const float *z, const float *bias, const float *gamma, const float *stats, float *dz, uint16_t *dz16, int lddz16, float *grads,
                           float *partial, int rows, int H, void *stream) {
  if (!dy || !z || !bias || !gamma || !stats || (!dz && !dz16) || !grads || !partial) return fail(TMJX_EINVAL, "null argument");
  if (rows < 1) return fail(TMJX_EINVAL, "rows must be >= 1");
  if (dz16 && (lddz16 < H || (lddz16 & 3) || ((uintptr_t)dz16 & 7))) return fail(TMJX_EINVAL, "tmjx_silu_ln_bwd_bf16: the output's rows must be 8-byte aligned and H wide");
  hipStream_t s = (hipStream_t)stream;
  const int nblk = (rows + BLK_ROWS_PER_BLOCK - 1) / BLK_ROWS_PER_BLOCK;
  unsigned short *o16 = (unsigned short *)dz16;
#define TMJX_BWD(V) do { if (o16) hipLaunchKernelGGL((k_silu_ln_bwd<V, true>), dim3(nblk), dim3(256), 0, s, dy, z, bias, gamma, stats, dz, partial, rows, o16, lddz16); \
                         else hipLaunchKernelGGL((k_silu_ln_bwd<V, false>), dim3(nblk), dim3(256), 0, s, dy, z, bias, gamma, stats, dz, partial, rows, o16, 0); } while (0)
  switch (H) { case 64: TMJX_BWD(1); break; case 128: TMJX_BWD(2); break; case 256: TMJX_BWD(4); break; case 512: TMJX_BWD(8); break;
               case 1024: TMJX_BWD(16); break; default: return fail(TMJX_EINVAL, "H must be 64, 128, 256, 512 or 1024"); }
#undef TMJX_BWD
  hipLaunchKernelGGL(k_colsum, dim3((3 * H + 31) / 32), dim3(256), 0, s, (const float *)partial, grads, nblk, 3 * H);
  return check_launch("k_silu_ln_bwd");
}
int tmjx_silu_ln_bwd(const float *dy, const float *z, const float *bias, const float *gamma, const float *stats, float *dz, float *grads,
                     float *partial, int rows, int H, void *stream) {
  if (!dz) return fail(TMJX_EINVAL, "null argument");
  return silu_ln_bwd_any(dy, z, bias, gamma, stats, dz, nullptr, 0, grads, partial, rows, H, stream);
}
int tmjx_silu_ln_bwd_bf16(const float *dy, const float *z, const float *bias, const float *gamma, const float *stats, uint16_t *dz16, int lddz16, float *grads,
                          float *partial, int rows, int H, void *stream) {
  if (!dz16) return fail(TMJX_EINVAL, "null argument");
  return silu_ln_bwd_any(dy, z, bias, gamma, stats, nullptr, dz16, lddz16, grads, partial, rows, H, stream);
}

int tmjx_gather_normalize(const float *src, const int64_t *idx, const float *mean, const float *std, float *out, int T, int R, int B,
                          int W, void *stream) {
  if (!src || !idx || !mean || !std || !out) return fail(TMJX_EINVAL, "null argument");
  if (T < 1 || R < 1 || B < 1 || W < 4 || (W & 3)) return fail(TMJX_EINVAL, "bad T / R / B / W (W must be a multiple of 4)");
  size_t total = (size_t)T * B * (W >> 2);
  int grid = (int)((total + 255) / 256 < 8192 ? (total + 255) / 256 : 8192);
  hipLaunchKernelGGL(k_gather_normalize, dim3(grid), dim3(256), 0, (hipStream_t)stream, src, (const long long *)idx, mean, std, out, T, R, B, W);
  return check_launch("k_gather_normalize");
}

static int launch_minibatch(const MinibatchGather &g, hipStream_t s) {
  if (!g.obs || !g.next_last || !g.raw_action || !g.scalar[0] || !g.scalar[1] || !g.scalar[2] || !g.scalar[3] || !g.idx || !g.mean || !g.stdv || !g.obs_n || !g.next_n ||
      !g.raw_action_g || !g.scalars_g)
    return fail(TMJX_EINVAL, "null argument");
  if (g.T < 1 || g.R < 1 || g.B < 1 || g.A < 1 || g.W < 4 || (g.W & 3)) return fail(TMJX_EINVAL, "bad T / R / B / A / W (W must be a multiple of 4)");
  if (g.eps && g.Z < 1) return fail(TMJX_EINVAL, "Z must be >= 1 with eps");
  const size_t nact = (size_t)g.T * g.B * g.A;
  const size_t total = (size_t)g.T * g.B * (g.W >> 2) + (size_t)g.B * (g.W >> 2) + nact + (size_t)4 * g.T * g.B + (g.eps ? ((size_t)g.T * g.B * g.Z + 3) / 4 : 0) +
                       (g.noise ? (nact + 3) / 4 : 0);
  const int grid = (int)((total + 255) / 256 < 8192 ? (total + 255) / 256 : 8192);
  hipLaunchKernelGGL(k_gather_minibatch, dim3(grid), dim3(256), 0, s, g);
  return check_launch("k_gather_minibatch");
}
int tmjx_gather_minibatch(const float *obs, const float *next_last, const float *raw_action, const float *log_prob, const float *reward, const float *discount,
                          const float *truncation, const int64_t *idx, const float *mean, const float *std, float *obs_n, float *next_n, float *raw_action_g,
                          float *scalars_g, int T, int R, int B, int W, int A, void *stream) {
  MinibatchGather g{obs, next_last, raw_action, {log_prob, reward, discount, truncation}, (const long long *)idx, mean, std, obs_n, next_n, raw_action_g, scalars_g,
                    nullptr, nullptr, nullptr, 0ull, T, R, B, W, A, 0, 0, nullptr, 0};
  return launch_minibatch(g, (hipStream_t)stream);
}
int tmjx_minibatch_begin(const tmjx_minibatch_t *m, void *stream) {
  if (!m) return fail(TMJX_EINVAL, "null argument");
  if ((m->eps || m->noise || m->advance) && !m->state) return fail(TMJX_EINVAL, "tmjx_minibatch_begin: draws / advance need the device state");
  MinibatchGather g{m->obs, m->next_last, m->raw_action, {m->log_prob, m->reward, m->discount, m->truncation}, (const long long *)m->perm, m->mean, m->std, m->obs_n,
                    m->next_n, m->raw_action_g, m->scalars_g, m->eps, m->noise, (long long *)m->state, (unsigned long long)m->seed, m->T, m->R, m->B, m->W, m->A,
                    m->Z, m->advance, nullptr, 0};
  return launch_minibatch(g, (hipStream_t)stream);
}
int tmjx_minibatch_begin_bf16(const tmjx_minibatch_t *m, uint16_t *obs_n16, int ld16, void *stream) {
  if (!m || !obs_n16) return fail(TMJX_EINVAL, "null argument");
  if ((m->eps || m->noise || m->advance) && !m->state) return fail(TMJX_EINVAL, "tmjx_minibatch_begin_bf16: draws / advance need the device state");
  if (ld16 < m->W || (ld16 & 3) || ((uintptr_t)obs_n16 & 7)) return fail(TMJX_EINVAL, "tmjx_minibatch_begin_bf16: the twin's rows must be 8-byte aligned and W wide");
  MinibatchGather g{m->obs, m->next_last, m->raw_action, {m->log_prob, m->reward, m->discount, m->truncation}, (const long long *)m->perm, m->mean, m->std, m->obs_n,
                    m->next_n, m->raw_action_g, m->scalars_g, m->eps, m->noise, (long long *)m->state, (unsigned long long)m->seed, m->T, m->R, m->B, m->W, m->A,
                    m->Z, m->advance, (unsigned short *)obs_n16, ld16};
  return launch_minibatch(g, (hipStream_t)stream);
}
int tmjx_philox4x32_10(const uint32_t *ctr_key_dev, uint32_t *out_dev, void *stream) {
  if (!ctr_key_dev || !out_dev) return fail(TMJX_EINVAL, "null argument");
  hipLaunchKernelGGL(k_philox_kat, dim3(1), dim3(64), 0, (hipStream_t)stream, ctr_key_dev, out_dev);
  return check_launch("k_philox_kat");
}

int tmjx_colsum_scratch_floats(int width) { return COLSUM_CHUNKS * width; }

int tmjx_colsum(const float *src, float *out, float *scratch, int rows, int width, void *stream) {
  if (!src || !out || !scratch) return fail(TMJX_EINVAL, "null argument");
  if (rows < 1 || width < 1) return fail(TMJX_EINVAL, "rows and width must be >= 1");
  hipStream_t s = (hipStream_t)stream;
  hipLaunchKernelGGL(k_colsum_rows, dim3((width + 31) / 32, COLSUM_CHUNKS), dim3(256), 0, s, src, scratch, rows, width);
  hipLaunchKernelGGL(k_colsum, dim3((width + 31) / 32), dim3(256), 0, s, (const float *)scratch, out, COLSUM_CHUNKS, width);
  return check_launch("k_colsum_rows");
}

int tmjx_colsum_grouped(const tmjx_colsum_problem_t *q, int n, void *stream) {
  if (!q || n < 1 || n > COLSUM_GROUP_MAX) return fail(TMJX_EINVAL, "tmjx_colsum_grouped: 1 .. 16 problems");
  ColsumGroup G;
  G.n = n;
  int blocks = 0;
  for (int i = 0; i < n; i++) {
    if (!q[i].partial || !q[i].out || q[i].rows < 1 || q[i].width < 1) return fail(TMJX_EINVAL, "tmjx_colsum_grouped: bad problem");
    G.p[i] = ColsumProblem{q[i].partial, q[i].out, q[i].rows, q[i].width, blocks};
    blocks += (q[i].width + 31) / 32;
  }
  hipLaunchKernelGGL(k_colsum_grouped, dim3(blocks), dim3(256), 0, (hipStream_t)stream, G);
  return check_launch("k_colsum_grouped");
}

int tmjx_adam_clip(float *param, const float *grad, float *exp_avg, float *exp_avg_sq, const float *grad_norm, long long n, float lr,
                   float beta1, float beta2, float eps, float bias_correction1, float bias_correction2, float max_norm, void *stream) {
  if (!param || !grad || !exp_avg || !exp_avg_sq || !grad_norm) return fail(TMJX_EINVAL, "null argument");
  if (n < 1 || !(bias_correction1 > 0.f) || !(bias_correction2 > 0.f) || !(max_norm > 0.f)) return fail(TMJX_EINVAL, "bad n / bias corrections / max_norm");
  int grid = (int)((n + 255) / 256 < 4096 ? (n + 255) / 256 : 4096);
  hipLaunchKernelGGL(k_adam_clip<false>, dim3(grid), dim3(256), 0, (hipStream_t)stream, param, grad, exp_avg, exp_avg_sq, grad_norm, n, lr, beta1, beta2, eps,
                     bias_correction1, bias_correction2, max_norm, (float *)nullptr);
  return check_launch("k_adam_clip");
}
int tmjx_adam_norm_floats(void) { return ADAM_NORM_PARTS; }
int tmjx_adam_clip_norm(float *param, const float *grad, float *exp_avg, float *exp_avg_sq, float *norm_scratch, float *norm_out, long long n, float lr,
                        float beta1, float beta2, float eps, float bias_correction1, float bias_correction2, float max_norm, void *stream) {
  if (!param || !grad || !exp_avg || !exp_avg_sq || !norm_scratch) return fail(TMJX_EINVAL, "null argument");
  if (n < 1 || !(bias_correction1 > 0.f) || !(bias_correction2 > 0.f) || !(max_norm > 0.f)) return fail(TMJX_EINVAL, "bad n / bias corrections / max_norm");
  if ((uintptr_t)grad & 15) return fail(TMJX_EINVAL, "tmjx_adam_clip_norm: the gradient buffer must be 16-byte aligned");
  hipStream_t s = (hipStream_t)stream;
  hipLaunchKernelGGL(k_grad_sumsq, dim3(ADAM_NORM_PARTS), dim3(256), 0, s, grad, n, norm_scratch);
  int grid = (int)((n + 255) / 256 < 4096 ? (n + 255) / 256 : 4096);
  hipLaunchKernelGGL(k_adam_clip<true>, dim3(grid), dim3(256), 0, s, param, grad, exp_avg, exp_avg_sq, (const float *)norm_scratch, n, lr, beta1, beta2, eps,
                     bias_correction1, bias_correction2, max_norm, norm_out);
  return check_launch("k_adam_clip(norm)");
}
int tmjx_adam_clip_norm_frozen(float *param, const float *grad, float *exp_avg, float *exp_avg_sq, float *norm_scratch, float *norm_out, long long n,
                               long long frozen_lo, long long frozen_hi, float lr, float beta1, float beta2, float eps, float bias_correction1,
                               float bias_correction2, float max_norm, void *stream) {
  if (!param || !grad || !exp_avg || !exp_avg_sq || !norm_scratch) return fail(TMJX_EINVAL, "tmjx_adam_clip_norm_frozen: null argument");
  if (n < 1 || !(bias_correction1 > 0.f) || !(bias_correction2 > 0.f) || !(max_norm > 0.f))
    return fail(TMJX_EINVAL, "tmjx_adam_clip_norm_frozen: bad n / bias corrections / max_norm");
  if ((uintptr_t)grad & 15) return fail(TMJX_EINVAL, "tmjx_adam_clip_norm_frozen: the gradient buffer must be 16-byte aligned");
  if (frozen_lo < 0 || frozen_lo > frozen_hi || frozen_hi > n)
    return fail(TMJX_EINVAL, "tmjx_adam_clip_norm_frozen: the frozen range must satisfy 0 <= lo <= hi <= n");
  if ((frozen_lo | frozen_hi) & 3)
    return fail(TMJX_EINVAL, "tmjx_adam_clip_norm_frozen: the frozen range's ends must be multiples of 4 (flat segments start on 16-byte boundaries)");
  hipStream_t s = (hipStream_t)stream;
  hipLaunchKernelGGL(k_grad_sumsq, dim3(ADAM_NORM_PARTS), dim3(256), 0, s, grad, n, norm_scratch);
  int grid = (int)((n + 255) / 256 < 4096 ? (n + 255) / 256 : 4096);
  hipLaunchKernelGGL(k_adam_clip_frozen, dim3(grid), dim3(256), 0, s, param, grad, exp_avg, exp_avg_sq, (const float *)norm_scratch, n, frozen_lo, frozen_hi,
                     lr, beta1, beta2, eps, bias_correction1, bias_correction2, max_norm, norm_out);
  return check_launch("k_adam_clip_frozen");
}

int tmjx_latent_concat(const float *fc2, const float *eps, const float *obs, float *x, int n, int Z, int obs_w, int ref_w,
                       int64_t obs_s0, int64_t obs_s1, const float *mean, const float *std, int x_stride, uint64_t seed, const int64_t *rng_state,
                       void *stream) {
  if (!fc2 || !obs || !x) return fail(TMJX_EINVAL, "null argument");
  if (!eps && !rng_state) return fail(TMJX_EINVAL, "tmjx_latent_concat: eps == NULL needs rng_state");
  if (n < 1 || Z < 1 || ref_w < 0 || obs_w < ref_w || x_stride < Z + obs_w - ref_w) return fail(TMJX_EINVAL, "bad sizes");
  size_t total = (size_t)n * x_stride;
  const size_t bt = n <= TMJX_SMALL_BATCH ? 64 : 256;
  int grid = (int)((total + bt - 1) / bt < 4096 ? (total + bt - 1) / bt : 4096);
  hipLaunchKernelGGL(k_latent_concat, dim3(grid), dim3((unsigned)bt), 0, (hipStream_t)stream, fc2, eps, obs, x, n, Z, obs_w, ref_w, (long long)obs_s0, (long long)obs_s1, mean, std, x_stride,
                     (unsigned long long)seed, (const long long *)rng_state);
  return check_launch("k_latent_concat");
}

static int launch_latent_concat_bwd(const float *dx, const float *eps, const float *fc2, const float *add, float *dfc2, int n, int Z, int dx_stride, void *stream) {
  if (!dx || !eps || !fc2 || !dfc2) return fail(TMJX_EINVAL, "null argument");
  if (n < 1 || Z < 1 || dx_stride < Z) return fail(TMJX_EINVAL, "bad sizes");
  size_t total = (size_t)n * Z;
  int grid = (int)((total + 255) / 256 < 4096 ? (total + 255) / 256 : 4096);
  hipLaunchKernelGGL(k_latent_concat_bwd, dim3(grid), dim3(256), 0, (hipStream_t)stream, dx, eps, fc2, dfc2, n, Z, dx_stride, add);
  return check_launch("k_latent_concat_bwd");
}
int tmjx_latent_concat_bwd(const float *dx, const float *eps, const float *fc2, float *dfc2, int n, int Z, int dx_stride, void *stream) {
  return launch_latent_concat_bwd(dx, eps, fc2, nullptr, dfc2, n, Z, dx_stride, stream);
}
int tmjx_latent_concat_bwd_add(const float *dx, const float *eps, const float *fc2, const float *add, float *dfc2, int n, int Z, int dx_stride, void *stream) {
  if (!add) return fail(TMJX_EINVAL, "null argument");
  return launch_latent_concat_bwd(dx, eps, fc2, add, dfc2, n, Z, dx_stride, stream);
}

int tmjx_sample_action(const float *logits, const float *noise, float *raw, float *action_t, float *logp, int n, int A, uint64_t seed,
                       int64_t *rng_state, void *stream) {
  if (!logits || !raw || !action_t || !logp) return fail(TMJX_EINVAL, "null argument");
  if (!noise && !rng_state) return fail(TMJX_EINVAL, "tmjx_sample_action: noise == NULL needs rng_state");
  if (n < 1 || A < 1) return fail(TMJX_EINVAL, "bad sizes");
  const int sbt = n <= TMJX_SMALL_BATCH ? 64 : PPO_BLOCK;
  hipLaunchKernelGGL(k_sample_action, dim3((n * PPO_G + sbt - 1) / sbt), dim3(sbt), 0, (hipStream_t)stream, logits, noise, raw, action_t, logp, n, A,
                     (unsigned long long)seed, (long long *)(noise ? nullptr : rng_state));
  return check_launch("k_sample_action");
}

int tmjx_linear_nolds_norm(const float *A, int64_t sa_row, int64_t sa_k, const float *W, const float *bias, float *C, int M, int N, int K,
                           const float *mean, const float *inv_std, void *stream) {
  if (!A || !W || !C || !mean || !inv_std) return fail(TMJX_EINVAL, "null argument");
  if (M < 1 || N < 1 || K < 1) return fail(TMJX_EINVAL, "bad sizes");
  const bool kmajor = sa_row == 1 && sa_k != 1;
  if (!kmajor && sa_k != 1) return fail(TMJX_EINVAL, "A must be row-major (sa_k == 1) or K-major (sa_row == 1)");
  if ((K & 3) || ((uintptr_t)W & 15) || ((uintptr_t)mean & 15) || ((uintptr_t)inv_std & 15) || (!kmajor && ((sa_row & 3) || ((uintptr_t)A & 15))))
    return fail(TMJX_EINVAL, "tmjx_linear_nolds_norm: K % 4 == 0 and 16-byte aligned operands");
  hipStream_t s = (hipStream_t)stream;
  dim3 g2((M + 31) / 32, (N + 31) / 32);
  if (kmajor) hipLaunchKernelGGL((k_linear_nolds_mfma<true>), g2, dim3(64), 0, s, A, (long long)sa_row, (long long)sa_k, W, bias, C, M, N, K, mean, inv_std);
  else hipLaunchKernelGGL((k_linear_nolds_mfma<false>), g2, dim3(64), 0, s, A, (long long)sa_row, (long long)sa_k, W, bias, C, M, N, K, mean, inv_std);
  return check_launch("k_linear_nolds_mfma(norm)");
}
int tmjx_linear_act_ok(const float *A, int64_t lda, const float *W, int ldw, int K) {
  return !(K & 3) && !((uintptr_t)A & 15) && !(lda & 3) && !((uintptr_t)W & 15) && !(ldw & 3) && lda >= K && ldw >= K;
}
int tmjx_linear_act(const float *A, int64_t lda, const float *W, int ldw, const float *bias, float *C, int M, int N, int K, const float *mean,
                    const float *inv_std, void *stream) {
  if (!A || !W || !C) return fail(TMJX_EINVAL, "null argument");
  if (M < 1 || N < 1 || K < 1) return fail(TMJX_EINVAL, "bad sizes");
  if (!tmjx_linear_act_ok(A, lda, W, ldw, K)) return fail(TMJX_EINVAL, "tmjx_linear_act: K % 4 == 0, row-major operands with 16-byte aligned rows");
  if ((mean || inv_std) && (!mean || !inv_std || (((uintptr_t)mean | (uintptr_t)inv_std) & 15))) return fail(TMJX_EINVAL, "tmjx_linear_act: mean and inv_std together, 16-byte aligned");
  hipStream_t s = (hipStream_t)stream;
  const int ncol = (N + ACT_BM - 1) / ACT_BM;
  const bool small = ((M + 63) / 64) * ncol < 128;
  if (small) {
    dim3 grid((M + 31) / 32, ncol);
    if (mean) hipLaunchKernelGGL((k_linear_act<true, 32>), grid, dim3(256), 0, s, A, (long long)lda, W, ldw, bias, C, M, N, K, mean, inv_std);
    else hipLaunchKernelGGL((k_linear_act<false, 32>), grid, dim3(256), 0, s, A, (long long)lda, W, ldw, bias, C, M, N, K, (const float *)nullptr, (const float *)nullptr);
  } else {
    dim3 grid((M + ACT_BM - 1) / ACT_BM, ncol);
    if (mean) hipLaunchKernelGGL((k_linear_act<true, 64>), grid, dim3(256), 0, s, A, (long long)lda, W, ldw, bias, C, M, N, K, mean, inv_std);
    else hipLaunchKernelGGL((k_linear_act<false, 64>), grid, dim3(256), 0, s, A, (long long)lda, W, ldw, bias, C, M, N, K, (const float *)nullptr, (const float *)nullptr);
  }
  return check_launch("k_linear_act");
}
int tmjx_linear_nolds(const float *A, int64_t sa_row, int64_t sa_k, const float *W, const float *bias, float *C, int M, int N, int K,
                      void *stream) {
  if (!A || !W || !C) return fail(TMJX_EINVAL, "null argument");
  if (M < 1 || N < 1 || K < 1) return fail(TMJX_EINVAL, "bad sizes");
  const bool kmajor = sa_row == 1 && sa_k != 1;
// ... 177 lines not shown
                                                             ln);
}
extern "C" {
int tmjx_gemm_nn_ln_bwd_ok(const float *dY, int ldy, const float *W, int ldw, int N) { return N == 256 && aligned16(dY, ldy) && aligned16(W, ldw); }
long long tmjx_gemm_nn_ln_bwd_partial_floats(int M, int N) { const int bm = 16 * gemm_mt(M, 1); return (long long)((M + bm - 1) / bm) * 3 * N; }
int tmjx_gemm_nn_ln_bwd(const float *dY, int ldy, const float *W, int ldw, const float *z, const float *bias, const float *gamma, const float *stats,
                        float *dz, float *partial, int M, int N, int K, void *stream) {
  if (!dY || !W || !z || !bias || !gamma || !stats || !dz || !partial) return fail(TMJX_EINVAL, "null argument");
  if (M < 1 || K < 1 || ldy < K || ldw < N) return fail(TMJX_EINVAL, "bad sizes / leading dimensions");
  if (!tmjx_gemm_nn_ln_bwd_ok(dY, ldy, W, ldw, N)) return fail(TMJX_EINVAL, "tmjx_gemm_nn_ln_bwd: N must be 256 and the operands' rows 16-byte aligned");
  GemmLN ln{gamma, nullptr, nullptr, const_cast<float *>(stats), 0.f, z, partial};
  if (gemm_mt(M, 1) == 2) return launch_gemm_ln_bwd<2>(dY, ldy, W, ldw, bias, dz, M, N, K, ln, (hipStream_t)stream);
  return launch_gemm_ln_bwd<5>(dY, ldy, W, ldw, bias, dz, M, N, K, ln, (hipStream_t)stream);
}
int tmjx_gemm_nn(const float *A, int lda, const float *W, int ldw, float *C, int ldc, int M, int N, int K, void *stream) {
  return gemm_act<false>(A, lda, W, ldw, nullptr, C, ldc, M, N, K, stream);
}
constexpr int DW_WGS = 256;
static void dw_split(int M, int N, int K, int *rows_per_split, int *S, int *ld_slab, int max_slabs = 0) {
  const int tiles = ((N + DW_BT - 1) / DW_BT) * ((K + DW_BT - 1) / DW_BT);
  int want = (DW_WGS + tiles - 1) / tiles;
  if (max_slabs > 0 && want > max_slabs) want = max_slabs;
  if (want < 1) want = 1;
  int rps = (((M + want - 1) / want) + DW_BM - 1) / DW_BM * DW_BM;
  if (rps < DW_BM) rps = DW_BM;
  *rows_per_split = rps;
  *S = (M + rps - 1) / rps;
  *ld_slab = ((K + DW_BT - 1) / DW_BT) * DW_BT + 4;
}
long long tmjx_gemm_dw_scratch_floats(int M, int N, int K) {
  if (M < 1 || N < 1 || K < 1) return 0;
  int rps, S, ld;
  dw_split(M, N, K, &rps, &S, &ld);
  return (long long)S * N * ld;
}
int tmjx_gemm_dw(const float *dY, int ldy, const float *X, int ldx, float *dW, float *db, float *scratch, int M, int N, int K, void *stream) {
  if (!dY || !X || !dW || !scratch) return fail(TMJX_EINVAL, "null argument");
  if (M < 1 || N < 1 || K < 1 || ldy < N || ldx < K) return fail(TMJX_EINVAL, "bad sizes / leading dimensions");
  int rps, S, ld;
  dw_split(M, N, K, &rps, &S, &ld);
  hipStream_t s = (hipStream_t)stream;
  const bool yv = aligned16(dY, ldy), xv = aligned16(X, ldx);
  int rc;
  if (yv && xv) rc = launch_gemm_dw<true, true>(dY, ldy, X, ldx, scratch, M, N, K, db ? 1 : 0, rps, S, ld, s);
  else if (yv) rc = launch_gemm_dw<true, false>(dY, ldy, X, ldx, scratch, M, N, K, db ? 1 : 0, rps, S, ld, s);
  else if (xv) rc = launch_gemm_dw<false, true>(dY, ldy, X, ldx, scratch, M, N, K, db ? 1 : 0, rps, S, ld, s);
  else rc = launch_gemm_dw<false, false>(dY, ldy, X, ldx, scratch, M, N, K, db ? 1 : 0, rps, S, ld, s);
  if (rc) return rc;
  const long long total = (long long)N * (K + (db ? 1 : 0));
  hipLaunchKernelGGL(k_dw_reduce, dim3((unsigned)((total + 255) / 256)), dim3(256), 0, s, (const float *)scratch, dW, db, S, N, K, db ? 1 : 0, ld, K);
  return check_launch("k_gemm_dw");
}

int tmjx_gemm_dw_grouped(const tmjx_dw_problem_t *probs, int n, void *stream) {
  if (!probs) return fail(TMJX_EINVAL, "null argument");
  if (n < 1 || n > DW_GROUP_MAX) return fail(TMJX_EINVAL, "1 .. 16 problems per group");
  DwGroup G;
  G.n = n;
  int wg = 0, red = 0;
  int all_tiles = 0;
  for (int i = 0; i < n; i++) all_tiles += ((probs[i].N + DW_BT - 1) / DW_BT) * ((probs[i].K + DW_BT - 1) / DW_BT);
  if (all_tiles < 1) all_tiles = 1;
  const int max_slabs = all_tiles <= 256 ? 256 / all_tiles : (1024 + all_tiles - 1) / all_tiles;
  for (int i = 0; i < n; i++) {
    const tmjx_dw_problem_t &q = probs[i];
    if (!q.dY || !q.X || !q.dW || !q.scratch) return fail(TMJX_EINVAL, "null pointer in a problem");
    if (q.M < 1 || q.N < 1 || q.K < 1 || q.ldy < q.N || q.ldx < q.K || q.lddw < q.K) return fail(TMJX_EINVAL, "bad sizes / leading dimensions in a problem");
    if (!aligned16(q.dY, q.ldy) || !aligned16(q.X, q.ldx)) return fail(TMJX_EINVAL, "grouped weight gradients need 16-byte aligned rows of dY and X");
    DwProblem &P = G.p[i];
    P.dY = q.dY; P.X = q.X; P.dW = q.dW; P.db = q.db; P.slabs = q.scratch;
    P.ldy = q.ldy; P.ldx = q.ldx; P.lddw = q.lddw; P.M = q.M; P.N = q.N; P.K = q.K;
    dw_split(q.M, q.N, q.K, &P.rows_per_split, &P.S, &P.ld_slab, max_slabs);
    P.tiles_n = (q.N + DW_BT - 1) / DW_BT; P.tiles_k = (q.K + DW_BT - 1) / DW_BT;
    P.wg_begin = wg; wg += P.tiles_n * P.tiles_k * P.S;
    P.red_begin = red; red += (int)(((long long)q.N * (q.K + (q.db ? 1 : 0)) + 255) / 256);
  }
  constexpr size_t lds = 2 * sizeof(float) * 2 * DW_BM * DW_LD;
  hipStream_t s = (hipStream_t)stream;
  const int rc = launch_lds<k_gemm_dw_grouped>("k_gemm_dw_grouped", dim3(wg), dim3(512), lds, s, G);
  if (rc) return rc;
  hipLaunchKernelGGL(k_dw_reduce_grouped, dim3(red), dim3(256), 0, s, G);
  return check_launch("k_gemm_dw_grouped");
}

int tmjx_rollout_store(const tmjx_rollout_store_t *q, void *stream) {
  if (!q) return fail(TMJX_EINVAL, "null argument");
  if (q->n < 1 || q->W < 0 || q->A < 0) return fail(TMJX_EINVAL, "bad sizes");
  if ((q->obs_dst0 || q->obs_dst1 || q->obs_dst2) && (!q->obs || q->W < 1)) return fail(TMJX_EINVAL, "observation destination without a source");
  if ((q->raw_dst && !q->raw) || (q->logp_dst && !q->logp) || (q->reward_dst && !q->reward) || (q->discount_dst && !q->done) || (q->trunc_dst && !q->trunc))
    return fail(TMJX_EINVAL, "destination without a source");
  RolloutStore s{q->obs, q->obs_dst0, q->obs_dst1, q->raw, q->raw_dst, q->logp, q->logp_dst, q->reward, q->reward_dst, q->done, q->discount_dst,
                 q->trunc, q->trunc_dst, q->n, q->W, q->A, q->obs_dst2};
  const int ny = (q->obs_dst0 || q->obs_dst1 || q->obs_dst2) ? (q->W + 15) / 16 : 0;
  hipLaunchKernelGGL(k_rollout_store, dim3((q->n + 63) / 64, ny + 1), dim3(64), 0, (hipStream_t)stream, s);
  return check_launch("k_rollout_store");
}

int tmjx_stats_scratch_floats(int W) { return STATS_SLABS * 2 * W; }

int tmjx_stats_sums(const float *src, const float *mean, float *sums, float *scratch, long long rows, int W, void *stream) {
  if (!src || !mean || !sums || !scratch) return fail(TMJX_EINVAL, "null argument");
  if (rows < 1 || W < 4 || (W & 3)) return fail(TMJX_EINVAL, "rows must be >= 1 and W a positive multiple of 4");
  if (((uintptr_t)src | (uintptr_t)mean | (uintptr_t)scratch) & 15) return fail(TMJX_EINVAL, "src, mean and scratch must be 16-byte aligned");
  hipStream_t s = (hipStream_t)stream;
  hipLaunchKernelGGL(k_stats_partial, dim3(((W >> 2) + 63) / 64, STATS_SLABS), dim3(256), 0, s, src, mean, scratch, rows, W);
  hipLaunchKernelGGL(k_colsum, dim3((2 * W + 31) / 32), dim3(256), 0, s, (const float *)scratch, sums, STATS_SLABS, 2 * W);
  return check_launch("k_stats_partial");
}

int tmjx_stats_apply(const float *sums, float n_added, float *count, float *mean, float *summed_variance, float *std, int W, float std_min,
                     float std_max, void *stream) {
  if (!sums || !count || !mean || !summed_variance || !std) return fail(TMJX_EINVAL, "null argument");
  if (W < 1 || !(n_added > 0.f)) return fail(TMJX_EINVAL, "W must be >= 1 and n_added > 0");
  hipStream_t s = (hipStream_t)stream;
  hipLaunchKernelGGL(k_stats_finalize, dim3((W + 255) / 256), dim3(256), 0, s, sums, n_added, count, mean, summed_variance, std, W, std_min, std_max);
  hipLaunchKernelGGL(k_stats_count, dim3(1), dim3(1), 0, s, count, n_added);
  return check_launch("k_stats_finalize");
}

int tmjx_stats_apply_pinned(const float *sums, float n_added, float *count, float *mean, float *summed_variance, float *std, int W, int pin_lo,
                            float std_min, float std_max, void *stream) {
  if (!sums || !count || !mean || !summed_variance || !std) return fail(TMJX_EINVAL, "tmjx_stats_apply_pinned: null argument");
  if (W < 1 || !(n_added > 0.f)) return fail(TMJX_EINVAL, "tmjx_stats_apply_pinned: W must be >= 1 and n_added > 0");
  if (pin_lo < 0 || pin_lo > W) return fail(TMJX_EINVAL, "tmjx_stats_apply_pinned: pin_lo must satisfy 0 <= pin_lo <= W");
  hipStream_t s = (hipStream_t)stream;
  hipLaunchKernelGGL(k_stats_finalize_pinned, dim3((W + 255) / 256), dim3(256), 0, s, sums, n_added, count, mean, summed_variance, std, W, pin_lo,
                     std_min, std_max);
  hipLaunchKernelGGL(k_stats_count, dim3(1), dim3(1), 0, s, count, n_added);
  return check_launch("k_stats_finalize_pinned");
}

int tmjx_debug_rows(const tmjx_model *m, const char *name, int *row0, int *count) {
  if (!m || !name || !row0 || !count) return fail(TMJX_EINVAL, "null argument");
  if (!strcmp(name, "k2_kernel")) {
    *row0 = m->rodent ? 1 : 0;
// ... 10 lines not shown
```

track_mjx_amd/hip.py:

```python
from __future__ import annotations

import ctypes as C
import os
import subprocess
from pathlib import Path

_PKG = Path(__file__).resolve().parent
SO_PATH = Path(os.environ.get("TMJX_SO", str(_PKG / "libtmjx_hip.so")))
CSRC = _PKG / "csrc"
SOURCES = (CSRC / "tmjx_hip.hip", CSRC / "tmjx_bf16.hip", CSRC / "tmjx_wave.hip", CSRC / "tmjx_chain.hip", CSRC / "tmjx_lstm.hip",
           CSRC / "tmjx_rollout.hip", CSRC / "tmjx_wave_sensors.hip", CSRC / "tmjx_wave_align.hip", CSRC / "tmjx_wave_rand.hip", CSRC / "tmjx_render.hip", CSRC / "tmjx_act.hip", CSRC / "tmjx_pca.hip", CSRC / "tmjx_pca_wide.hip", CSRC / "tmjx_readout.hip", CSRC / "tmjx_intervene.hip", CSRC / "tmjx_kmeans.hip", CSRC / "tmjx_hmm.hip", CSRC / "tmjx_spectrogram.hip", CSRC / "tmjx_arhmm.hip", CSRC / "tmjx_tsne.hip", CSRC / "tmjx_compare.hip", CSRC / "tmjx_jacobian.hip", CSRC / "tmjx_lstm_jacobian.hip", CSRC / "tmjx_lstm_tangent.hip")
SOURCE_FLAGS = {"tmjx_wave.hip": ("-mllvm", "-disable-machine-licm"),
                "tmjx_wave_sensors.hip": ("-mllvm", "-disable-machine-licm"),
                "tmjx_wave_rand.hip": ("-mllvm", "-disable-machine-licm"),
                "tmjx_jacobian.hip": ("-ffp-contract=off",),
                "tmjx_lstm_jacobian.hip": ("-ffp-contract=off",),
                "tmjx_lstm_tangent.hip": ("-ffp-contract=off",)}


class TmjxError(RuntimeError):
    pass


class Layout(C.Structure):
    _fields_ = [(n, C.c_int32) for n in (
        "nq", "nv", "nu", "nbody", "ncon", "nefc", "obs_size", "ref_obs_size", "n_metrics", "window",
        "qpos", "qvel", "act", "qacc_warmstart", "time", "xpos", "xmat_torso", "qfrc_actuator",
        "prev_ctrl", "action_buffer", "done", "steps_f", "first_phys", "first_obs", "first_prev_ctrl", "state_rows",
        "i_clip_idx", "i_start_frame", "i_buffer_index", "i_nan_count", "istate_rows", "ws_rows")]


class Minibatch(C.Structure):
    _fields_ = ([(k, C.c_void_p) for k in ("obs", "next_last", "raw_action", "log_prob", "reward", "discount", "truncation", "perm", "mean", "std", "obs_n", "next_n",
                                           "raw_action_g", "scalars_g", "eps", "noise", "state")] + [("seed", C.c_uint64)] +
                [(k, C.c_int32) for k in ("T", "R", "B", "W", "A", "Z", "advance")])


class ColsumProblem(C.Structure):
    _fields_ = [("partial", C.c_void_p), ("out", C.c_void_p), ("rows", C.c_int32), ("width", C.c_int32)]


class DwProblem(C.Structure):
    _fields_ = [("dY", C.c_void_p), ("X", C.c_void_p), ("dW", C.c_void_p), ("db", C.c_void_p), ("scratch", C.c_void_p),
                ("ldy", C.c_int32), ("ldx", C.c_int32), ("lddw", C.c_int32), ("M", C.c_int32), ("N", C.c_int32), ("K", C.c_int32)]


class BdwProblem(C.Structure):
    _fields_ = [("dY", C.c_void_p), ("X", C.c_void_p), ("dW", C.c_void_p), ("db", C.c_void_p), ("scratch", C.c_void_p),
                ("y_is_f32", C.c_int32), ("x_is_f32", C.c_int32), ("ldy", C.c_int32), ("ldx", C.c_int32), ("lddw", C.c_int32), ("M", C.c_int32), ("N", C.c_int32), ("K", C.c_int32)]


class RolloutStore(C.Structure):
    _fields_ = [(k, C.c_void_p) for k in ("obs", "obs_dst0", "obs_dst1", "raw", "raw_dst", "logp", "logp_dst", "reward", "reward_dst", "done", "discount_dst",
                                          "trunc", "trunc_dst")] + [(k, C.c_int32) for k in ("n", "W", "A")] + [("obs_dst2", C.c_void_p)]


class Bf16Shadow(C.Structure):
    _fields_ = [("src", C.c_void_p), ("dst", C.c_void_p), ("dst_t", C.c_void_p), ("N", C.c_int32), ("K", C.c_int32), ("ld_src", C.c_int32),
                ("ld_dst", C.c_int32), ("ld_dst_t", C.c_int32)]


class ChainLayer(C.Structure):
    _fields_ = [(k, C.c_void_p) for k in ("W", "bias", "gamma", "beta", "z", "y", "stats")] + [("K", C.c_int32), ("ldw", C.c_int32)]


class ChainFwd(C.Structure):
    _fields_ = [("A", C.c_void_p), ("lda", C.c_int32), ("M", C.c_int32), ("n_hidden", C.c_int32), ("epi", C.c_int32), ("hidden", ChainLayer * 4),
                ("Wf", C.c_void_p), ("bf", C.c_void_p), ("outf", C.c_void_p), ("Nf", C.c_int32), ("ldwf", C.c_int32), ("ldof", C.c_int32), ("eps", C.c_float), ("rows_alloc", C.c_int32),
                ("prof", C.c_void_p)]


CHAIN_MAX_HIDDEN = 4


class DecoderBlock(C.Structure):
    _fields_ = [(k, C.c_void_p) for k in ("W", "bias", "gamma", "beta")] + [("width", C.c_int32), ("ldw", C.c_int32)]


class DecoderAct(C.Structure):
    _fields_ = [("latents", C.c_void_p), ("ldz", C.c_int32), ("obs", C.c_void_p), ("obs_s0", C.c_int64), ("obs_s1", C.c_int64), ("mean", C.c_void_p),
                ("std", C.c_void_p), ("n", C.c_int32), ("Z", C.c_int32), ("obs_w", C.c_int32), ("ref_w", C.c_int32), ("n_blocks", C.c_int32),
                ("block", DecoderBlock * CHAIN_MAX_HIDDEN), ("Wf", C.c_void_p), ("bf", C.c_void_p), ("ldwf", C.c_int32), ("A", C.c_int32), ("eps", C.c_float),
                ("action_t", C.c_void_p), ("ctrl", C.c_void_p), ("logits", C.c_void_p), ("ldl", C.c_int32)]


class PolicyAct(C.Structure):
    _fields_ = ([("obs", C.c_void_p), ("ldo", C.c_int64)] + [(k, C.c_void_p) for k in ("mean", "inv_std", "nmean", "nstd")] +
                [(k, C.c_int32) for k in ("n", "K0", "Z", "obs_w", "ref_w", "A", "n_enc", "n_dec")] +
                [("enc", DecoderBlock * CHAIN_MAX_HIDDEN), ("dec", DecoderBlock * CHAIN_MAX_HIDDEN), ("W2", C.c_void_p), ("b2", C.c_void_p),
                 ("ldw2", C.c_int32), ("ldwh", C.c_int32), ("Wh", C.c_void_p), ("bh", C.c_void_p), ("eps", C.c_void_p), ("noise", C.c_void_p),
                 ("seed", C.c_uint64), ("rng_state", C.c_void_p), ("ln_eps", C.c_float), ("pad_", C.c_int32)] +
                [(k, C.c_void_p) for k in ("fc2", "logits", "raw", "action_t", "logp")])
# ... 151 lines not shown

_i, _i64, _u64, _f, _d, _vp, _s, _P = C.c_int, C.c_int64, C.c_uint64, C.c_float, C.c_double, C.c_void_p, C.c_char_p, C.POINTER
SIGNATURES = {
    "tmjx_model_create": ([_s, C.c_size_t, _P(_vp)], _i),
    "tmjx_model_destroy": ([_vp], None),
    "tmjx_layout": ([_vp, _P(Layout)], _i),
    "tmjx_clips_upload": ([_vp] * 6 + [_i, _i], _i),
    "tmjx_reset": ([_vp] * 9 + [_i, _vp], _i),
    "tmjx_step": ([_vp] * 10 + [_i, _vp], _i),
    "tmjx_physics": ([_vp, _vp, _vp, _i, _vp, _i, _vp], _i),
    "tmjx_physics_step": ([_vp] * 4 + [_i, _vp], _i),
    "tmjx_forward": ([_vp, _vp, _vp, _i, _vp], _i),
    "tmjx_reward_obs": ([_vp] * 10 + [_i, _vp], _i),
    "tmjx_reward_frame": ([_vp] * 14 + [_i, _vp], _i),
    "tmjx_gae": ([_vp] * 5 + [_f, _f, _vp, _vp, _i, _i, _vp], _i),
    "tmjx_ppo_scratch_floats": ([_i, _i], _i),
    "tmjx_ppo_loss": ([_P(PpoCfg)] + [_vp] * 16, _i),
    "tmjx_ppo_loss_phases": ([_P(PpoCfg)] + [_vp] * 15 + [_i, _vp], _i),
    "tmjx_silu_ln_partial_floats": ([_i, _i], _i),
    "tmjx_silu_ln_fwd": ([_vp] * 6 + [_i, _i, _f, _vp], _i),
    "tmjx_silu_ln_bwd": ([_vp] * 8 + [_i, _i, _vp], _i),
    "tmjx_silu_ln_fwd_bf16": ([_vp] * 5 + [_i, _vp, _i, _i, _f, _vp], _i),
    "tmjx_silu_ln_bwd_bf16": ([_vp] * 6 + [_i, _vp, _vp, _i, _i, _vp], _i),
    "tmjx_minibatch_begin_bf16": ([_P(Minibatch), _vp, _i, _vp], _i),
    "tmjx_gather_normalize": ([_vp] * 5 + [_i] * 4 + [_vp], _i),
    "tmjx_latent_concat": ([_vp] * 4 + [_i] * 4 + [_i64, _i64, _vp, _vp, _i, _u64, _vp, _vp], _i),
    "tmjx_latent_concat_bwd": ([_vp] * 4 + [_i, _i, _i, _vp], _i),
    "tmjx_latent_concat_bwd_add": ([_vp] * 5 + [_i, _i, _i, _vp], _i),
    "tmjx_sample_action": ([_vp] * 5 + [_i, _i, _u64, _vp, _vp], _i),
    "tmjx_linear_nolds": ([_vp, _i64, _i64, _vp, _vp, _vp, _i, _i, _i, _vp], _i),
    "tmjx_linear_act": ([_vp, _i64, _vp, _i, _vp, _vp, _i, _i, _i, _vp, _vp, _vp], _i),
    "tmjx_linear_act_ok": ([_vp, _i64, _vp, _i, _i], _i),
    "tmjx_linear_nolds_norm": ([_vp, _i64, _i64, _vp, _vp, _vp, _i, _i, _i, _vp, _vp, _vp], _i),
    "tmjx_linear_nolds_bf16": ([_vp, _i64, _i64, _vp, _i, _vp, _vp, _i, _i, _i, _vp, _vp, _vp], _i),
    "tmjx_adam_clip": ([_vp] * 5 + [_i64] + [_f] * 7 + [_vp], _i),
    "tmjx_adam_clip_norm": ([_vp] * 6 + [_i64] + [_f] * 7 + [_vp], _i),
    "tmjx_adam_clip_norm_frozen": ([_vp] * 6 + [_i64, _i64, _i64] + [_f] * 7 + [_vp], _i),
    "tmjx_adam_norm_floats": ([], _i),
    "tmjx_colsum_scratch_floats": ([_i], _i),
    "tmjx_colsum": ([_vp, _vp, _vp, _i, _i, _vp], _i),
    "tmjx_gather_minibatch": ([_vp] * 14 + [_i] * 5 + [_vp], _i),
    "tmjx_minibatch_begin": ([_P(Minibatch), _vp], _i),
    "tmjx_philox4x32_10": ([_vp, _vp, _vp], _i),
    "tmjx_gemm_nt": ([_vp, _i, _vp, _i, _vp, _vp] + [_i] * 4 + [_vp], _i),
    "tmjx_gemm_nt_silu_ln": ([_vp, _i, _vp, _i] + [_vp] * 5 + [_i, _vp, _i, _i, _i, _f, _vp], _i),
    "tmjx_gemm_nt_silu_ln_ok": ([_vp, _i, _vp, _i, _i], _i),
    "tmjx_gemm_nn": ([_vp, _i, _vp, _i, _vp] + [_i] * 4 + [_vp], _i),
    "tmjx_colsum_grouped": ([_P(ColsumProblem), _i, _vp], _i),
    "tmjx_gemm_nn_ln_bwd": ([_vp, _i, _vp, _i] + [_vp] * 6 + [_i, _i, _i, _vp], _i),
    "tmjx_gemm_nn_ln_bwd_ok": ([_vp, _i, _vp, _i, _i], _i),
    "tmjx_gemm_nn_ln_bwd_partial_floats": ([_i, _i], _i64),
    "tmjx_gemm_dw": ([_vp, _i, _vp, _i, _vp, _vp, _vp, _i, _i, _i, _vp], _i),
    "tmjx_gemm_dw_grouped": ([_P(DwProblem), _i, _vp], _i),
    "tmjx_gemm_dw_scratch_floats": ([_i, _i, _i], _i64),
    "tmjx_set_wrappers": ([_vp, _i, _i], _i),
    "tmjx_set_action_repeat": ([_vp, _i], _i),
    "tmjx_stats_scratch_floats": ([_i], _i),
    "tmjx_stats_sums": ([_vp] * 4 + [_i64, _i, _vp], _i),
    "tmjx_stats_apply": ([_vp, _f] + [_vp] * 4 + [_i, _f, _f, _vp], _i),
    "tmjx_stats_apply_pinned": ([_vp, _f] + [_vp] * 4 + [_i, _i, _f, _f, _vp], _i),
    "tmjx_rollout_store": ([_P(RolloutStore), _vp], _i),
    "tmjx_clips_share": ([_vp, _vp], _i),
    "tmjx_gemm_nt_silu": ([_vp, _i, _vp, _i, _vp, _vp, _vp] + [_i] * 4 + [_vp], _i),
    "tmjx_gemm_nt_silu_ok": ([_vp, _i, _vp, _i], _i),
    "tmjx_silu_fwd": ([_vp, _vp, _vp, _i64, _i, _vp], _i),
    "tmjx_silu_bwd": ([_vp] * 4 + [_i64, _i, _vp], _i),
    "tmjx_gemm_nn_silu_bwd_ok": ([_vp, _i, _vp, _i], _i),
    "tmjx_gemm_nn_silu_bwd": ([_vp, _i, _vp, _i, _vp, _vp, _vp, _i, _i, _i, _vp], _i),
    "tmjx_silu_bwd_rank1": ([_vp] * 5 + [_i64, _i, _vp], _i),
    "tmjx_head_dw_scratch_floats": ([_i, _i], _i64),
    "tmjx_head_dw": ([_vp, _vp, _i, _vp, _vp, _vp, _i, _i, _vp], _i),
    "tmjx_head_fwd_ok": ([_vp, _i, _vp, _i], _i),
    "tmjx_head_fwd": ([_vp, _i, _vp, _vp, _vp, _i, _i, _vp], _i),
    "tmjx_bf16_shadow": ([_P(Bf16Shadow), _i, _vp], _i),
    "tmjx_bgemm_nt": ([_vp, _i, _i, _vp, _i, _vp, _vp] + [_i] * 4 + [_vp], _i),
    "tmjx_bgemm_dw": ([_vp, _i, _i, _vp, _i, _i, _vp, _i, _vp, _vp, _i, _i, _i, _vp], _i),
    "tmjx_bgemm_dw_grouped": ([_P(BdwProblem), _i, _i, _vp], _i),
    "tmjx_bgemm_dw_scratch_floats": ([_i, _i, _i], _i64),
    "tmjx_bgemm_row_tile_ok": ([_i], _i),
    "tmjx_bf16_z_bytes": ([], _i),
    "tmjx_bgemm_partial_floats": ([_i, _i, _i], _i64),
    "tmjx_bgemm_ln_fwd": ([_vp, _i, _i, _vp, _i] + [_vp] * 4 + [_i, _vp, _i, _vp, _i, _i, _i, _f, _vp], _i),
    "tmjx_bgemm_ln_bwd": ([_vp, _i, _i, _vp, _i, _vp, _i] + [_vp] * 4 + [_i, _vp, _i, _i, _i, _vp], _i),
    "tmjx_bgemm_silu_fwd": ([_vp, _i, _i, _vp, _i, _vp, _vp, _i, _vp, _i, _vp] + [_i] * 4 + [_vp], _i),
    "tmjx_bgemm_silu_bwd": ([_vp, _i, _i, _vp, _i, _vp, _i, _vp, _vp, _i, _vp, _i, _i, _i, _vp], _i),
    "tmjx_bf_silu_bwd": ([_vp, _i, _vp, _i, _vp, _vp, _i, _vp, _i, _i, _vp], _i),
    "tmjx_bf_silu_bwd_rank1": ([_vp, _vp, _vp, _i, _vp, _vp, _i, _vp, _i, _i, _vp], _i),
    "tmjx_chain_rows": ([_i], _i),
    "tmjx_chain_fwd_ok": ([_P(ChainFwd)], _i),
    "tmjx_chain_fwd": ([_P(ChainFwd), _vp], _i),
    "tmjx_chain_bwd_ok": ([_P(ChainBwd)], _i),
    "tmjx_chain_bwd": ([_P(ChainBwd), _vp], _i),
    "tmjx_lstm_hidden_ok": ([_i], _i),
    "tmjx_lstm_seq_fwd": ([_P(LstmFwd), _vp], _i),
    "tmjx_lstm_seq_bwd": ([_P(LstmBwd), _vp], _i),
    "tmjx_record_check": ([_P(RecordStream), _i, _i, _i], _i),
    "tmjx_record_step": ([_vp] + [_i] * 4 + [_vp], _i),
    "tmjx_latent_concat_det": ([_vp, _i, _vp, _i64, _i64, _vp, _vp, _vp, _i, _vp] + [_i] * 5 + [_vp], _i),
    "tmjx_action_mode": ([_vp, _i, _vp, _vp, _i, _i, _vp], _i),
    "tmjx_decoder_input": ([_vp, _i, _vp, _i64, _i64, _vp, _vp, _vp] + [_i] * 5 + [_vp], _i),
    "tmjx_decoder_act_ok": ([_P(DecoderAct)], _i),
    "tmjx_decoder_act": ([_P(DecoderAct), _vp], _i),
    "tmjx_lstm_decoder_act_ok": ([_P(LstmDecoderAct)], _i),
    "tmjx_lstm_decoder_act": ([_P(LstmDecoderAct), _vp], _i),
    "tmjx_policy_act_ok": ([_P(PolicyAct)], _i),
    "tmjx_policy_act": ([_P(PolicyAct), _vp], _i),
# ... 180 lines not shown
```

Baseline: 1.723 million.

## Fuse minibatch gather into decoder input and merge grad reductions into one finish kernel

The minibatch gather now writes the normalized obs slice straight into a padded decoder-input buffer. A new latent-sample kernel then fills only the latent columns in place, which removes the separate latent-concat copy. On the backward side, the LayerNorm gamma/beta/bias column sums and the dW slab reductions are merged into a single grad_finish launch that writes directly into param.grad, and the head dW also writes in place. This cuts kernel launches and intermediate buffers in the SGD phase, at the cost of more conditional code paths and alignment requirements.

```diff
diff --git a/include/tmjx.h b/include/tmjx.h
--- a/include/tmjx.h
+++ b/include/tmjx.h
@@ -118,6 +118,8 @@
 } tmjx_minibatch_t;
 int tmjx_minibatch_begin(const tmjx_minibatch_t *mb, void *stream);
 int tmjx_minibatch_begin_bf16(const tmjx_minibatch_t *mb, uint16_t *obs_n16, int ld16, void *stream);
+int tmjx_gather_minibatch_x_ok(const float *x, int x_stride, int W, int ref_w, int Z);
+int tmjx_gather_minibatch_x(const tmjx_minibatch_t *mb, float *x, int x_stride, int ref_w, int Z, void *stream);
 int tmjx_philox4x32_10(const uint32_t *ctr_key_dev, uint32_t *out_dev, void *stream);
 
 int tmjx_latent_concat_bwd(const float *dx, const float *eps, const float *fc2, float *dfc2, int n, int Z, int dx_stride, void *stream);
@@ -129,6 +131,11 @@
                        void *stream);
 int tmjx_sample_action(const float *logits, const float *noise, float *raw, float *action_t, float *logp, int n, int A, uint64_t seed,
                        int64_t *rng_state, void *stream);
+int tmjx_latent_sample_ok(const float *fc2, const float *eps, const float *x, int Z, int x_stride);
+int tmjx_latent_sample(const float *fc2, const float *eps, float *x, int n, int Z, int x_stride, uint64_t seed, const int64_t *rng_state, void *stream);
+int tmjx_latent_sample_bwd(const float *dx, const float *eps, const float *fc2, float *dfc2, int n, int Z, int dx_stride, void *stream);
+int tmjx_latent_sample_bwd_add(const float *dx, const float *eps, const float *fc2, const float *add, float *dfc2, int n, int Z, int dx_stride,
+                               void *stream);
 
 int tmjx_linear_act_ok(const float *A, int64_t lda, const float *W, int ldw, int K);
 int tmjx_linear_act(const float *A, int64_t lda, const float *W, int ldw, const float *bias, float *C, int M, int N, int K,
@@ -208,6 +215,9 @@
   int32_t ldy, ldx, lddw, M, N, K;
 } tmjx_dw_problem_t;
 int tmjx_gemm_dw_grouped(const tmjx_dw_problem_t *problems, int n, void *stream);
+typedef struct tmjx_colsum_ld_problem_t { const float *partial; float *out; int32_t rows, width, ld, pad_; } tmjx_colsum_ld_problem_t;
+int tmjx_gemm_dw_slabs_grouped(const tmjx_dw_problem_t *problems, int n, void *stream);
+int tmjx_grad_finish(const tmjx_dw_problem_t *problems, int n, const tmjx_colsum_ld_problem_t *sums, int n_sums, void *stream);
 
 typedef struct tmjx_bf16_shadow_t {
   const float *src;
diff --git a/track_mjx_amd/agent/losses.py b/track_mjx_amd/agent/losses.py
--- a/track_mjx_amd/agent/losses.py
+++ b/track_mjx_amd/agent/losses.py
@@ -5,6 +5,7 @@
 import torch
 
 from .. import hip as _hip
+from . import networks as _networks
 from .networks import NormalTanh
 
 
@@ -54,7 +55,7 @@
 
 
 def minibatch_begin(buf: dict, perm: torch.Tensor, state: torch.Tensor, seed: int, normalizer, latents: int, advance: bool = True,
-                    obs16: torch.Tensor | None = None) -> dict:
+                    obs16: torch.Tensor | None = None, ref_w: int | None = None) -> dict:
     obs, nxt, act = buf["observation"], buf["next_observation_last"], buf["raw_action"]
     T, R, W = obs.shape
     B, A = int(buf["_B"]), act.shape[-1]
@@ -73,6 +74,14 @@
             assert obs16.dtype == torch.bfloat16 and obs16.shape[0] == T * B and obs16.shape[1] >= W and obs16.is_contiguous()
             _hip.check(_hip.lib().tmjx_minibatch_begin_bf16(C.byref(m), C.c_void_p(obs16.data_ptr()), obs16.shape[1], stream), "tmjx_minibatch_begin_bf16")
             out["observation_normalized_bf16"] = obs16
+        elif ref_w is not None and _networks.SGD_SMALL_KERNELS and 0 <= ref_w <= W:
+            wd = latents + W - ref_w
+            x = torch.empty((T * B, (wd + 3) // 4 * 4), **f32)
+            if _hip.lib().tmjx_gather_minibatch_x_ok(C.c_void_p(x.data_ptr()), x.shape[1], W, ref_w, latents):
+                _hip.check(_hip.lib().tmjx_gather_minibatch_x(C.byref(m), C.c_void_p(x.data_ptr()), x.shape[1], ref_w, latents, stream), "tmjx_gather_minibatch_x")
+                out["decoder_input"] = x
+            else:
+                _hip.check(_hip.lib().tmjx_minibatch_begin(C.byref(m), stream), "tmjx_minibatch_begin")
         else:
             _hip.check(_hip.lib().tmjx_minibatch_begin(C.byref(m), stream), "tmjx_minibatch_begin")
     return out
@@ -128,6 +137,7 @@
     cfg_of = lambda A_, Z_: _hip.PpoCfg(T, B, A_, Z_, reward_scaling, discounting, gae_lambda, clipping_epsilon, entropy_cost, kl_weight,
                                         int(normalize_advantage), int(acc_out is not None))
     f32 = lambda a: a.detach().contiguous().float()
+    xk = {"x_buf": data["decoder_input"]} if "decoder_input" in data else {}
     if side_stream is not None:
         cur = torch.cuda.current_stream(dev)
         with torch.no_grad():
@@ -142,12 +152,12 @@
             if phased:
                 with torch.no_grad():
                     bl, bs = f32(baseline), f32(bootstrap)
-        logits, fc2 = policy(obs, eps=data.get("latent_eps"), return_fc2=True)
+        logits, fc2 = policy(obs, eps=data.get("latent_eps"), return_fc2=True, **xk)
         if not phased:
             cur.wait_stream(side_stream)
         baseline.record_stream(cur); bootstrap.record_stream(cur)
     else:
-        logits, fc2 = policy(obs, eps=data.get("latent_eps"), return_fc2=True)
+        logits, fc2 = policy(obs, eps=data.get("latent_eps"), return_fc2=True, **xk)
         baseline = value(obs)
         with torch.no_grad():
             bootstrap = value(nxt)
diff --git a/track_mjx_amd/agent/networks.py b/track_mjx_amd/agent/networks.py
--- a/track_mjx_amd/agent/networks.py
+++ b/track_mjx_amd/agent/networks.py
@@ -248,6 +248,7 @@
 
     def __enter__(self):
         self.problems, self.keep, self.colsums = [], [], []
+        self.sums = []
         self.bproblems = []
         self.seen: set = set()
         deferred_weight_grads.active = self
@@ -276,8 +277,34 @@
         self.problems.append((dy2, x2, gw, gb))
         return gw, gb
 
+    def dests(self, params):
+        if not SGD_SMALL_KERNELS or any(p.grad is None or p.grad.shape != p.shape or not p.grad.is_contiguous() or id(p) in self.seen for p in params):
+            return None
+        self.seen.update(id(p) for p in params)
+        return [p.grad for p in params]
+
+    def add_ln_sums(self, partial, nblk, gamma, beta, bias):
+        if len(self.sums) + 3 > 16:
+            return None
+        views = self.dests((gamma, beta, bias))
+        if views is None:
+            return None
+        N = gamma.numel()
+        self.sums += [(partial, j * N, v, nblk, N, 3 * N) for j, v in enumerate(views)]
+        return views
+
     def launch(self):
         from .. import hip as _hip
+        if SGD_SMALL_KERNELS:
+            self.sums = [(pt, 0, g, nb, wd, wd) for pt, g, nb, wd in self.colsums] + self.sums
+            self.colsums = []
+            while len(self.sums) > 16:
+                self._launch_problems([], self.sums[:16])
+                self.sums = self.sums[16:]
+            self._launch_problems(self.problems, self.sums)
+            self.problems, self.sums = [], []
+            self._launch_bproblems()
+            return
         if self.colsums:
             dev = self.colsums[0][0].device
             arr = (_hip.ColsumProblem * len(self.colsums))(*[_hip.ColsumProblem(pt.data_ptr(), g.data_ptr(), nb, wd) for pt, g, nb, wd in self.colsums])
@@ -310,9 +337,13 @@
             _launch("tmjx_bgemm_dw_grouped", dev, arr, len(grp), 0)
             self.keep += [scratch] + [t for q in grp for t in q[:2]]
 
-    def _launch_problems(self, problems):
+    def _launch_problems(self, problems, sums=None):
         from .. import hip as _hip
         if not problems:
+            if sums:
+                arr = (_hip.ColsumLdProblem * len(sums))(*[_hip.ColsumLdProblem(pt.data_ptr() + 4 * c0, o.data_ptr(), nb, wd, ld, 0) for pt, c0, o, nb, wd, ld in sums])
+                _launch("tmjx_grad_finish", sums[0][0].device, None, 0, arr, len(sums))
+                self.keep += [t for q in sums for t in (q[0], q[2])]
             return
         L = _hip.lib()
         dev = problems[0][0].device
@@ -324,7 +355,13 @@
             arr[i] = _hip.DwProblem(dy.data_ptr(), x.data_ptr(), gw.data_ptr(), gb.data_ptr() if gb is not None else None,
                                     scratch.data_ptr() + 4 * off, dy.stride(0), x.stride(0), gw.stride(0), dy.shape[0], dy.shape[1], x.shape[1])
             off += (sizes[i] + 3) // 4 * 4
-        _launch("tmjx_gemm_dw_grouped", dev, arr, len(problems))
+        if sums is None:
+            _launch("tmjx_gemm_dw_grouped", dev, arr, len(problems))
+        else:
+            sarr = (_hip.ColsumLdProblem * max(len(sums), 1))(*[_hip.ColsumLdProblem(pt.data_ptr() + 4 * c0, o.data_ptr(), nb, wd, ld, 0) for pt, c0, o, nb, wd, ld in sums])
+            _launch("tmjx_gemm_dw_slabs_grouped", dev, arr, len(problems))
+            _launch("tmjx_grad_finish", dev, arr, len(problems), sarr, len(sums))
+            self.keep += [t for q in sums for t in (q[0], q[2])]
         self.keep += [scratch] + [t for q in problems for t in q[:2]]
 
 
@@ -613,7 +650,8 @@
             g = dout.reshape(-1)
             g = g if g.is_contiguous() else g.contiguous()
             K = wf.shape[1]
-            dwh, dbh = torch.empty((1, K), dtype=torch.float32, device=dev), torch.empty(1, dtype=torch.float32, device=dev)
+            into = d.dests((last.lin.weight, last.lin.bias)) if d is not None else None
+            dwh, dbh = into if into is not None else (torch.empty((1, K), dtype=torch.float32, device=dev), torch.empty(1, dtype=torch.float32, device=dev))
             scratch = torch.empty(int(Lh.tmjx_head_dw_scratch_floats(M, K)), dtype=torch.float32, device=dev)
             _launch("tmjx_head_dw", dev, _p(g), _p(y_last), y_last.stride(0), _p(dwh), _p(dbh), _p(scratch), M, K)
             grads[(len(layers) - 1, 0)], grads[(len(layers) - 1, 1)] = dwh, dbh
@@ -631,7 +669,10 @@
             blocks = [(P[l][0], saved[l][0], P[l][1]) for l in range(len(hid) - 1, -1, -1)]
         want_dx = ctx.needs_input_grad[0]
         cols = (x2.shape[1] if ctx.dx_cols is None else int(ctx.dx_cols)) if want_dx else None
-        dzs, partials, dx = chain_bwd(g, wf, blocks, kind, P[0][0] if want_dx else None, cols, dx_ld=x2.shape[1] if want_dx else None)
+        dx_ld = (x2.stride(0) if SGD_SMALL_KERNELS and x2.stride(0) % 4 == 0 and x2.stride(0) >= x2.shape[1] else x2.shape[1]) if want_dx else None
+        dzs, partials, dx = chain_bwd(g, wf, blocks, kind, P[0][0] if want_dx else None, cols, dx_ld=dx_ld)
+        if dx is not None:
+            dx = dx[:, :x2.shape[1]]
         for i, dz in enumerate(dzs):
             l = len(hid) - 1 - i
             L = hid[l]
@@ -639,8 +680,12 @@
             if kind == "ln":
                 got = d.try_add(dz, xin, L.lin.weight, None) if d is not None else None
                 grads[(l, 0)] = got[0] if got is not None else gemm_dw(dz, xin, False)[0]
+                nblk = partials[i].numel() // 768
+                views = d.add_ln_sums(partials[i], nblk, L.norm.weight, L.norm.bias, L.lin.bias) if d is not None else None
+                if views is not None:
+                    grads[(l, 2)], grads[(l, 3)], grads[(l, 1)] = views
+                    continue
                 g3 = torch.empty((3, 256), dtype=torch.float32, device=dev)
-                nblk = partials[i].numel() // 768
                 if d is not None and len(d.colsums) < 16:
                     d.colsums.append((partials[i], g3, nblk, 768))
                 else:
@@ -1057,15 +1102,55 @@
     def backward(ctx, dx):
         fc2, eps = ctx.saved_tensors
         n, Z = eps.shape
-        dx = dx.contiguous()
+        dx = dx if dx.dim() == 2 and dx.stride(1) == 1 and dx.stride(0) >= Z else dx.contiguous()
         dfc2 = torch.empty_like(fc2)
         add = ctx.handle.take() if ctx.handle is not None else None
         if add is not None and (add.shape != fc2.shape or not add.is_contiguous()):
             raise RuntimeError("_LatentConcatFn: the pending fc2 gradient does not fit this forward pass")
         if add is None:
-            _launch("tmjx_latent_concat_bwd", fc2.device, _p(dx), _p(eps), _p(fc2), _p(dfc2), n, Z, dx.shape[1])
+            _launch("tmjx_latent_concat_bwd", fc2.device, _p(dx), _p(eps), _p(fc2), _p(dfc2), n, Z, dx.stride(0))
         else:
-            _launch("tmjx_latent_concat_bwd_add", fc2.device, _p(dx), _p(eps), _p(fc2), _p(add), _p(dfc2), n, Z, dx.shape[1])
+            _launch("tmjx_latent_concat_bwd_add", fc2.device, _p(dx), _p(eps), _p(fc2), _p(add), _p(dfc2), n, Z, dx.stride(0))
+        return dfc2, None, None, None, None
+
+
+SGD_SMALL_KERNELS = True
+
+
+def _latent_sample_ok(fc2, eps, x_buf, n, Z, wd) -> bool:
+    from .. import hip as _hip
+    return (SGD_SMALL_KERNELS and x_buf is not None and x_buf.is_cuda and x_buf.dtype == torch.float32 and x_buf.dim() == 2 and x_buf.is_contiguous()
+            and tuple(x_buf.shape) == (n, (wd + 3) // 4 * 4) and fc2.is_contiguous() and eps.is_contiguous()
+            and bool(_hip.lib().tmjx_latent_sample_ok(_p(fc2), _p(eps), _p(x_buf), Z, x_buf.shape[1])))
+
+
+class _LatentSampleFn(torch.autograd.Function):
+
+    @staticmethod
+    def forward(ctx, fc2, eps, holder, wd, handle=None):
+        ctx.handle = handle
+        n, Z = eps.shape
+        x = holder[0]
+        _launch("tmjx_latent_sample", fc2.device, _p(fc2), _p(eps), _p(x), n, Z, x.shape[1], 0, None)
+        ctx.save_for_backward(fc2, eps)
+        return x[:, :wd]
+
+    @staticmethod
+    def backward(ctx, dx):
+        fc2, eps = ctx.saved_tensors
+        n, Z = eps.shape
+        dfc2 = torch.empty_like(fc2)
+        add = ctx.handle.take() if ctx.handle is not None else None
+        if add is not None and (add.shape != fc2.shape or not add.is_contiguous()):
+            raise RuntimeError("_LatentSampleFn: the pending fc2 gradient does not fit this forward pass")
+        fast = dx.dim() == 2 and dx.stride(1) == 1 and dx.stride(0) % 4 == 0 and dx.stride(0) >= Z and dx.data_ptr() % 16 == 0 and (add is None or add.data_ptr() % 16 == 0)
+        if not fast:
+            dx = dx if dx.dim() == 2 and dx.stride(1) == 1 and dx.stride(0) >= Z else dx.contiguous()
+        name = "tmjx_latent_sample_bwd" if fast else "tmjx_latent_concat_bwd"
+        if add is None:
+            _launch(name, fc2.device, _p(dx), _p(eps), _p(fc2), _p(dfc2), n, Z, dx.stride(0))
+        else:
+            _launch(name + "_add", fc2.device, _p(dx), _p(eps), _p(fc2), _p(add), _p(dfc2), n, Z, dx.stride(0))
         return dfc2, None, None, None, None
 
 
@@ -1109,7 +1194,8 @@
         dec[0].dx_cols = latents
         self.head = _dense(d, 2 * action_size)
 
-    def forward(self, obs: torch.Tensor, eps: torch.Tensor | None = None, deterministic: bool = False, return_fc2: bool = False):
+    def forward(self, obs: torch.Tensor, eps: torch.Tensor | None = None, deterministic: bool = False, return_fc2: bool = False,
+                x_buf: torch.Tensor | None = None):
         traj = obs[..., :self.reference_obs_size]
         prev, self.latent_grad_handle = getattr(self, "latent_grad_handle", None), None
         if prev is not None and prev.pending:
@@ -1138,7 +1224,12 @@
             if eps is None:
                 eps = torch.randn_like(mean)
             handle = LatentGradHandle(fc2.reshape(-1, fc2.shape[-1])) if (fc2.requires_grad and fc2.is_contiguous()) else None
-            x = _LatentConcatFn.apply(fc2.reshape(-1, fc2.shape[-1]), eps.reshape(-1, self.latents), obs.reshape(-1, obs.shape[-1]), self.reference_obs_size, handle)
+            f2, e2 = fc2.reshape(-1, fc2.shape[-1]), eps.reshape(-1, self.latents)
+            wd = self.latents + obs.shape[-1] - self.reference_obs_size
+            if _latent_sample_ok(f2, e2, x_buf, f2.shape[0], self.latents, wd):
+                x = _LatentSampleFn.apply(f2, e2, (x_buf,), wd, handle)
+            else:
+                x = _LatentConcatFn.apply(f2, e2, obs.reshape(-1, obs.shape[-1]), self.reference_obs_size, handle)
             self.latent_grad_handle = handle
             x = x.view(*lead, x.shape[-1])
             if chains:
diff --git a/track_mjx_amd/agent/ppo.py b/track_mjx_amd/agent/ppo.py
--- a/track_mjx_amd/agent/ppo.py
+++ b/track_mjx_amd/agent/ppo.py
@@ -635,7 +635,8 @@
         fused_gather = self.dev.type == "cuda" and self.normalize_observations and self.buf["observation"].shape[-1] % 4 == 0
         if idx is None:
             data = _losses.minibatch_begin({**self.buf, "_B": self.local_batch}, self._perm_static, self._mb_state, self._noise_seed, self.normalizer,
-                                           self.policy.latents, obs16=self._obs16)
+                                           self.policy.latents, obs16=self._obs16,
+                                           ref_w=self.policy.reference_obs_size if isinstance(self.policy, IntentionPolicy) else None)
         elif fused_gather and all(v.is_contiguous() for v in self.buf.values()):
             data = _losses.gather_minibatch(self.buf, idx, self.normalizer)
         else:
diff --git a/track_mjx_amd/csrc/gemm_kernels.h b/track_mjx_amd/csrc/gemm_kernels.h
--- a/track_mjx_amd/csrc/gemm_kernels.h
+++ b/track_mjx_amd/csrc/gemm_kernels.h
@@ -714,4 +714,19 @@
   const DwProblem &P = G.p[i];
   dw_reduce_elem(P.slabs, P.dW, P.db, P.S, P.N, P.K, P.db != nullptr, P.ld_slab, P.lddw, (long long)(blockIdx.x - P.red_begin) * 256 + threadIdx.x);
 }
-#endif
+__global__ __launch_bounds__(256) void k_grad_finish(const DwGroup G, const ColsumLdGroup Q, int red) {
+  __shared__ float lds[8][33];
+  if ((int)blockIdx.x < red) {
+    int i = 0;
+    for (int j = 1; j < G.n; j++) if ((int)blockIdx.x >= G.p[j].red_begin) i = j;
+    const DwProblem &P = G.p[i];
+    dw_reduce_elem(P.slabs, P.dW, P.db, P.S, P.N, P.K, P.db != nullptr, P.ld_slab, P.lddw, (long long)(blockIdx.x - P.red_begin) * 256 + threadIdx.x);
+  } else {
+    const int b = (int)blockIdx.x - red;
+    int i = 0;
+    for (int j = 1; j < Q.n; j++) if (b >= Q.p[j].blk_begin) i = j;
+    const ColsumLdProblem &P = Q.p[i];
+    colsum_block(P.partial, P.out, P.nblk, P.width, P.ld, b - P.blk_begin, lds);
+  }
+}
+#endif
diff --git a/track_mjx_amd/csrc/ppo_kernels.h b/track_mjx_amd/csrc/ppo_kernels.h
--- a/track_mjx_amd/csrc/ppo_kernels.h
+++ b/track_mjx_amd/csrc/ppo_kernels.h
@@ -686,7 +686,9 @@
   int T, R, B, W, A, Z, advance;
   unsigned short *obs_n16; int ld16;
 };
-__global__ __launch_bounds__(256) void k_gather_minibatch(MinibatchGather g) {
+struct MinibatchX { float *x; int x_stride, ref_w, Z, quad; };
+template <bool XOUT>
+__device__ __forceinline__ void gather_minibatch_body(MinibatchGather g, MinibatchX X) {
   const int w4 = g.W >> 2;
   const unsigned long long ctr = g.state ? (unsigned long long)g.state[0] : 0ull;
   const long long *idx = g.idx + (g.state ? g.state[1] * (long long)g.B : 0ll);
@@ -706,6 +708,16 @@
       const float4 o = {(v.x - m.x) / s.x, (v.y - m.y) / s.y, (v.z - m.z) / s.z, (v.w - m.w) / s.w};
       reinterpret_cast<float4 *>((nx ? g.next_n : g.obs_n) + tb * g.W)[c] = o;
       if (!nx && g.obs_n16) *reinterpret_cast<uint2 *>(g.obs_n16 + tb * g.ld16 + 4 * c) = uint2{silu_ln_pack(o.x, o.y), silu_ln_pack(o.z, o.w)};
+      if (XOUT && !nx) {
+        float *xr = X.x + tb * (size_t)X.x_stride;
+        const int k0 = 4 * c, d = X.Z - X.ref_w;
+        if (X.quad && k0 >= X.ref_w) *reinterpret_cast<float4 *>(xr + k0 + d) = o;
+        else {
+          if (k0 >= X.ref_w) *reinterpret_cast<float2 *>(xr + k0 + d) = float2{o.x, o.y}; else if (k0 + 1 >= X.ref_w) xr[k0 + 1 + d] = o.y;
+          if (k0 + 2 >= X.ref_w) *reinterpret_cast<float2 *>(xr + k0 + 2 + d) = float2{o.z, o.w}; else if (k0 + 3 >= X.ref_w) xr[k0 + 3 + d] = o.w;
+        }
+        if (c == w4 - 1) for (int p = g.W + d; p < X.x_stride; p++) xr[p] = 0.f;
+      }
     } else if (i < e1) {
       const size_t j = i - e0;
       const int c = (int)(j % g.A);
@@ -744,6 +756,8 @@
     }
   }
 }
+__global__ __launch_bounds__(256) void k_gather_minibatch(MinibatchGather g) { gather_minibatch_body<false>(g, MinibatchX{nullptr, 0, 0, 0, 0}); }
+__global__ __launch_bounds__(256) void k_gather_minibatch_x(MinibatchGather g, MinibatchX X) { gather_minibatch_body<true>(g, X); }
 __global__ void k_philox_kat(const unsigned *ctr_key, unsigned *out) {
   if (threadIdx.x == 0) tm_philox4x32_10(ctr_key[0], ctr_key[1], ctr_key[2], ctr_key[3], ctr_key[4], ctr_key[5], out);
 }
@@ -773,6 +787,43 @@
     if (add) { gm = add[e * 2 * Z + c] + gm; gv = add[e * 2 * Z + Z + c] + gv; }
     dfc2[e * 2 * Z + c] = gm;
     dfc2[e * 2 * Z + Z + c] = gv;
+  }
+}
+__global__ __launch_bounds__(256) void k_latent_sample(const float *__restrict__ fc2, const float *__restrict__ eps, float *__restrict__ x, unsigned total, int Z,
+                                                       int x_stride, unsigned long long seed, const long long *__restrict__ rng_state) {
+  const unsigned z4 = (unsigned)Z >> 2;
+  const unsigned long long ctr = rng_state ? (unsigned long long)rng_state[0] : 0ull;
+  for (unsigned i = blockIdx.x * 256u + threadIdx.x; i < total; i += gridDim.x * 256u) {
+    const unsigned e = i / z4, c = 4u * (i - e * z4);
+    const float *row = fc2 + (size_t)e * 2 * Z;
+    const float4 m = *reinterpret_cast<const float4 *>(row + c), lv = *reinterpret_cast<const float4 *>(row + Z + c);
+    float ep[4];
+    if (eps) { const float4 t = *reinterpret_cast<const float4 *>(eps + (size_t)e * Z + c); ep[0] = t.x; ep[1] = t.y; ep[2] = t.z; ep[3] = t.w; }
+    else tm_normal4(seed, ctr, 2u, (unsigned)(((size_t)e * Z + c) >> 2), ep);
+    *reinterpret_cast<float4 *>(x + (size_t)e * x_stride + c) =
+        float4{tm_latent_sample(ep[0], lv.x, m.x), tm_latent_sample(ep[1], lv.y, m.y), tm_latent_sample(ep[2], lv.z, m.z), tm_latent_sample(ep[3], lv.w, m.w)};
+  }
+}
+__global__ __launch_bounds__(256) void k_latent_sample_bwd(const float *__restrict__ dx, const float *__restrict__ eps, const float *__restrict__ fc2,
+                                                           float *__restrict__ dfc2, unsigned total, int Z, int dx_stride, const float *__restrict__ add) {
+  const unsigned z4 = (unsigned)Z >> 2;
+  for (unsigned i = blockIdx.x * 256u + threadIdx.x; i < total; i += gridDim.x * 256u) {
+    const unsigned e = i / z4, c = 4u * (i - e * z4);
+    const size_t r2 = (size_t)e * 2 * Z;
+    const float4 g4 = *reinterpret_cast<const float4 *>(dx + (size_t)e * dx_stride + c), e4 = *reinterpret_cast<const float4 *>(eps + (size_t)e * Z + c),
+                 l4 = *reinterpret_cast<const float4 *>(fc2 + r2 + Z + c);
+    const float g[4] = {g4.x, g4.y, g4.z, g4.w}, ep[4] = {e4.x, e4.y, e4.z, e4.w}, lv[4] = {l4.x, l4.y, l4.z, l4.w};
+    float gm[4], gv[4];
+#pragma unroll
+    for (int k = 0; k < 4; k++) { gm[k] = g[k]; gv[k] = g[k] * ep[k] * (0.5f * expf(0.5f * lv[k])); }
+    if (add) {
+      const float4 am = *reinterpret_cast<const float4 *>(add + r2 + c), av = *reinterpret_cast<const float4 *>(add + r2 + Z + c);
+      const float a0[4] = {am.x, am.y, am.z, am.w}, a1[4] = {av.x, av.y, av.z, av.w};
+#pragma unroll
+      for (int k = 0; k < 4; k++) { gm[k] = a0[k] + gm[k]; gv[k] = a1[k] + gv[k]; }
+    }
+    *reinterpret_cast<float4 *>(dfc2 + r2 + c) = float4{gm[0], gm[1], gm[2], gm[3]};
+    *reinterpret_cast<float4 *>(dfc2 + r2 + Z + c) = float4{gv[0], gv[1], gv[2], gv[3]};
   }
 }
 __global__ __launch_bounds__(PPO_BLOCK) void k_sample_action(const float *__restrict__ logits, const float *__restrict__ noise, float *__restrict__ raw,
@@ -959,25 +1010,30 @@
 #define COLSUM_GROUP_MAX 16
 struct ColsumProblem { const float *partial; float *out; int nblk, width, blk_begin; };
 struct ColsumGroup { ColsumProblem p[COLSUM_GROUP_MAX]; int n; };
+__device__ __forceinline__ void colsum_block(const float *__restrict__ partial, float *__restrict__ out, int nblk, int width, int ld, int block, float (*lds)[33]) {
+  const int cx = threadIdx.x & 31, ry = threadIdx.x >> 5, col = block * 32 + cx;
+  float acc[8] = {0.f, 0.f, 0.f, 0.f, 0.f, 0.f, 0.f, 0.f};
+  if (col < width) {
+    int k = ry;
+    for (; k + 56 < nblk; k += 64) {
+#pragma unroll
+      for (int u = 0; u < 8; u++) acc[u] += partial[(size_t)(k + 8 * u) * ld + col];
+    }
+    for (; k < nblk; k += 8) acc[0] += partial[(size_t)k * ld + col];
+  }
+  lds[ry][cx] = ((acc[0] + acc[1]) + (acc[2] + acc[3])) + ((acc[4] + acc[5]) + (acc[6] + acc[7]));
+  __syncthreads();
+  if (ry == 0 && col < width) { float s = 0.f; for (int j = 0; j < 8; j++) s += lds[j][cx]; out[col] = s; }
+}
 __global__ __launch_bounds__(256) void k_colsum_grouped(const ColsumGroup G) {
   __shared__ float lds[8][33];
   int i = 0;
   for (int j = 1; j < G.n; j++) if ((int)blockIdx.x >= G.p[j].blk_begin) i = j;
   const ColsumProblem &P = G.p[i];
-  const int cx = threadIdx.x & 31, ry = threadIdx.x >> 5, col = (blockIdx.x - P.blk_begin) * 32 + cx;
-  float acc[8] = {0.f, 0.f, 0.f, 0.f, 0.f, 0.f, 0.f, 0.f};
-  if (col < P.width) {
-    int k = ry;
-    for (; k + 56 < P.nblk; k += 64) {
-#pragma unroll
-      for (int u = 0; u < 8; u++) acc[u] += P.partial[(size_t)(k + 8 * u) * P.width + col];
-    }
-    for (; k < P.nblk; k += 8) acc[0] += P.partial[(size_t)k * P.width + col];
-  }
-  lds[ry][cx] = ((acc[0] + acc[1]) + (acc[2] + acc[3])) + ((acc[4] + acc[5]) + (acc[6] + acc[7]));
-  __syncthreads();
-  if (ry == 0 && col < P.width) { float s = 0.f; for (int j = 0; j < 8; j++) s += lds[j][cx]; P.out[col] = s; }
-}
+  colsum_block(P.partial, P.out, P.nblk, P.width, P.width, blockIdx.x - P.blk_begin, lds);
+}
+struct ColsumLdProblem { const float *partial; float *out; int nblk, width, ld, blk_begin; };
+struct ColsumLdGroup { ColsumLdProblem p[COLSUM_GROUP_MAX]; int n; };
 
 #define STATS_SLABS 512
 __global__ __launch_bounds__(256) void k_stats_partial(const float *__restrict__ src, const float *__restrict__ mean, float *__restrict__ partial,
diff --git a/track_mjx_amd/csrc/tmjx_hip.hip b/track_mjx_amd/csrc/tmjx_hip.hip
--- a/track_mjx_amd/csrc/tmjx_hip.hip
+++ b/track_mjx_amd/csrc/tmjx_hip.hip
@@ -783,7 +783,7 @@
   return check_launch("k_gather_normalize");
 }
 
-static int launch_minibatch(const MinibatchGather &g, hipStream_t s) {
+static int launch_minibatch(const MinibatchGather &g, hipStream_t s, const MinibatchX *X = nullptr) {
   if (!g.obs || !g.next_last || !g.raw_action || !g.scalar[0] || !g.scalar[1] || !g.scalar[2] || !g.scalar[3] || !g.idx || !g.mean || !g.stdv || !g.obs_n || !g.next_n ||
       !g.raw_action_g || !g.scalars_g)
     return fail(TMJX_EINVAL, "null argument");
@@ -793,6 +793,10 @@
   const size_t total = (size_t)g.T * g.B * (g.W >> 2) + (size_t)g.B * (g.W >> 2) + nact + (size_t)4 * g.T * g.B + (g.eps ? ((size_t)g.T * g.B * g.Z + 3) / 4 : 0) +
                        (g.noise ? (nact + 3) / 4 : 0);
   const int grid = (int)((total + 255) / 256 < 8192 ? (total + 255) / 256 : 8192);
+  if (X) {
+    hipLaunchKernelGGL(k_gather_minibatch_x, dim3(grid), dim3(256), 0, s, g, *X);
+    return check_launch("k_gather_minibatch_x");
+  }
   hipLaunchKernelGGL(k_gather_minibatch, dim3(grid), dim3(256), 0, s, g);
   return check_launch("k_gather_minibatch");
 }
@@ -819,6 +823,22 @@
                     m->next_n, m->raw_action_g, m->scalars_g, m->eps, m->noise, (long long *)m->state, (unsigned long long)m->seed, m->T, m->R, m->B, m->W, m->A,
                     m->Z, m->advance, (unsigned short *)obs_n16, ld16};
   return launch_minibatch(g, (hipStream_t)stream);
+}
+int tmjx_gather_minibatch_x_ok(const float *x, int x_stride, int W, int ref_w, int Z) {
+  return x && !((uintptr_t)x & 15) && W >= 4 && !(W & 3) && Z >= 1 && ref_w >= 0 && ref_w <= W && !((ref_w - Z) & 1) && !(x_stride & 3) &&
+         (long long)x_stride >= (long long)Z + W - ref_w;
+}
+int tmjx_gather_minibatch_x(const tmjx_minibatch_t *m, float *x, int x_stride, int ref_w, int Z, void *stream) {
+  if (!m || !x) return fail(TMJX_EINVAL, "null argument");
+  if ((m->eps || m->noise || m->advance) && !m->state) return fail(TMJX_EINVAL, "tmjx_gather_minibatch_x: draws / advance need the device state");
+  if (m->eps && m->Z != Z) return fail(TMJX_EINVAL, "tmjx_gather_minibatch_x: eps is drawn [T B mb->Z]: Z must equal mb->Z");
+  if (!tmjx_gather_minibatch_x_ok(x, x_stride, m->W, ref_w, Z))
+    return fail(TMJX_EINVAL, "tmjx_gather_minibatch_x: x must be 16-byte aligned with x_stride % 4 == 0 and >= Z + W - ref_w, 0 <= ref_w <= W, Z >= 1 and ref_w - Z even");
+  MinibatchGather g{m->obs, m->next_last, m->raw_action, {m->log_prob, m->reward, m->discount, m->truncation}, (const long long *)m->perm, m->mean, m->std, m->obs_n,
+                    m->next_n, m->raw_action_g, m->scalars_g, m->eps, m->noise, (long long *)m->state, (unsigned long long)m->seed, m->T, m->R, m->B, m->W, m->A,
+                    m->Z, m->advance, nullptr, 0};
+  const MinibatchX X{x, x_stride, ref_w, Z, ((ref_w - Z) & 3) == 0};
+  return launch_minibatch(g, (hipStream_t)stream, &X);
 }
 int tmjx_philox4x32_10(const uint32_t *ctr_key_dev, uint32_t *out_dev, void *stream) {
   if (!ctr_key_dev || !out_dev) return fail(TMJX_EINVAL, "null argument");
@@ -922,6 +942,39 @@
   return launch_latent_concat_bwd(dx, eps, fc2, add, dfc2, n, Z, dx_stride, stream);
 }
 
+static bool a16(const void *p) { return !((uintptr_t)p & 15); }
+int tmjx_latent_sample_ok(const float *fc2, const float *eps, const float *x, int Z, int x_stride) {
+  return fc2 && x && Z >= 4 && !(Z & 3) && x_stride >= Z && !(x_stride & 3) && a16(fc2) && a16(eps) && a16(x);
+}
+int tmjx_latent_sample(const float *fc2, const float *eps, float *x, int n, int Z, int x_stride, uint64_t seed, const int64_t *rng_state, void *stream) {
+  if (!fc2 || !x) return fail(TMJX_EINVAL, "null argument");
+  if (!eps && !rng_state) return fail(TMJX_EINVAL, "tmjx_latent_sample: eps == NULL needs rng_state");
+  if (n < 1 || (long long)n * (Z >> 2) > 0x7fffffffll) return fail(TMJX_EINVAL, "tmjx_latent_sample: bad n");
+  if (!tmjx_latent_sample_ok(fc2, eps, x, Z, x_stride))
+    return fail(TMJX_EINVAL, "tmjx_latent_sample: Z and x_stride must be multiples of 4, x_stride >= Z, and fc2, eps, x 16-byte aligned");
+  const unsigned total = (unsigned)n * (unsigned)(Z >> 2);
+  const unsigned grid = (total + 255) / 256 < 4096 ? (total + 255) / 256 : 4096;
+  hipLaunchKernelGGL(k_latent_sample, dim3(grid), dim3(256), 0, (hipStream_t)stream, fc2, eps, x, total, Z, x_stride, (unsigned long long)seed, (const long long *)rng_state);
+  return check_launch("k_latent_sample");
+}
+static int launch_latent_sample_bwd(const float *dx, const float *eps, const float *fc2, const float *add, float *dfc2, int n, int Z, int dx_stride, void *stream) {
+  if (!dx || !eps || !fc2 || !dfc2) return fail(TMJX_EINVAL, "null argument");
+  if (n < 1 || (long long)n * (Z >> 2) > 0x7fffffffll) return fail(TMJX_EINVAL, "tmjx_latent_sample_bwd: bad n");
+  if (Z < 4 || (Z & 3) || dx_stride < Z || (dx_stride & 3) || !a16(dx) || !a16(eps) || !a16(fc2) || !a16(add) || !a16(dfc2))
+    return fail(TMJX_EINVAL, "tmjx_latent_sample_bwd: Z and dx_stride must be multiples of 4, dx_stride >= Z, and every array 16-byte aligned");
+  const unsigned total = (unsigned)n * (unsigned)(Z >> 2);
+  const unsigned grid = (total + 255) / 256 < 4096 ? (total + 255) / 256 : 4096;
+  hipLaunchKernelGGL(k_latent_sample_bwd, dim3(grid), dim3(256), 0, (hipStream_t)stream, dx, eps, fc2, dfc2, total, Z, dx_stride, add);
+  return check_launch("k_latent_sample_bwd");
+}
+int tmjx_latent_sample_bwd(const float *dx, const float *eps, const float *fc2, float *dfc2, int n, int Z, int dx_stride, void *stream) {
+  return launch_latent_sample_bwd(dx, eps, fc2, nullptr, dfc2, n, Z, dx_stride, stream);
+}
+int tmjx_latent_sample_bwd_add(const float *dx, const float *eps, const float *fc2, const float *add, float *dfc2, int n, int Z, int dx_stride, void *stream) {
+  if (!add) return fail(TMJX_EINVAL, "null argument");
+  return launch_latent_sample_bwd(dx, eps, fc2, add, dfc2, n, Z, dx_stride, stream);
+}
+
 int tmjx_sample_action(const float *logits, const float *noise, float *raw, float *action_t, float *logp, int n, int A, uint64_t seed,
                        int64_t *rng_state, void *stream) {
   if (!logits || !raw || !action_t || !logp) return fail(TMJX_EINVAL, "null argument");
@@ -1205,12 +1258,11 @@
   return check_launch("k_gemm_dw");
 }
 
-int tmjx_gemm_dw_grouped(const tmjx_dw_problem_t *probs, int n, void *stream) {
+static int dw_group(const tmjx_dw_problem_t *probs, int n, DwGroup &G, int &wg, int &red) {
   if (!probs) return fail(TMJX_EINVAL, "null argument");
   if (n < 1 || n > DW_GROUP_MAX) return fail(TMJX_EINVAL, "1 .. 16 problems per group");
-  DwGroup G;
   G.n = n;
-  int wg = 0, red = 0;
+  wg = 0; red = 0;
   int all_tiles = 0;
   for (int i = 0; i < n; i++) all_tiles += ((probs[i].N + DW_BT - 1) / DW_BT) * ((probs[i].K + DW_BT - 1) / DW_BT);
   if (all_tiles < 1) all_tiles = 1;
@@ -1228,12 +1280,50 @@
     P.wg_begin = wg; wg += P.tiles_n * P.tiles_k * P.S;
     P.red_begin = red; red += (int)(((long long)q.N * (q.K + (q.db ? 1 : 0)) + 255) / 256);
   }
+  return TMJX_OK;
+}
+static int launch_dw_slabs(const DwGroup &G, int wg, hipStream_t s) {
   constexpr size_t lds = 2 * sizeof(float) * 2 * DW_BM * DW_LD;
-  hipStream_t s = (hipStream_t)stream;
-  const int rc = launch_lds<k_gemm_dw_grouped>("k_gemm_dw_grouped", dim3(wg), dim3(512), lds, s, G);
+  return launch_lds<k_gemm_dw_grouped>("k_gemm_dw_grouped", dim3(wg), dim3(512), lds, s, G);
+}
+int tmjx_gemm_dw_grouped(const tmjx_dw_problem_t *probs, int n, void *stream) {
+  DwGroup G;
+  int wg, red;
+  int rc = dw_group(probs, n, G, wg, red);
+  if (rc) return rc;
+  hipStream_t s = (hipStream_t)stream;
+  rc = launch_dw_slabs(G, wg, s);
   if (rc) return rc;
   hipLaunchKernelGGL(k_dw_reduce_grouped, dim3(red), dim3(256), 0, s, G);
   return check_launch("k_gemm_dw_grouped");
+}
+int tmjx_gemm_dw_slabs_grouped(const tmjx_dw_problem_t *probs, int n, void *stream) {
+  DwGroup G;
+  int wg, red;
+  const int rc = dw_group(probs, n, G, wg, red);
+  if (rc) return rc;
+  return launch_dw_slabs(G, wg, (hipStream_t)stream);
+}
+int tmjx_grad_finish(const tmjx_dw_problem_t *probs, int n, const tmjx_colsum_ld_problem_t *sums, int n_sums, void *stream) {
+  DwGroup G;
+  int wg = 0, red = 0;
+  G.n = 0;
+  if (n != 0) {
+    const int rc = dw_group(probs, n, G, wg, red);
+    if (rc) return rc;
+  }
+  if (n_sums < 0 || n_sums > COLSUM_GROUP_MAX || (n_sums && !sums) || (n == 0 && n_sums < 1)) return fail(TMJX_EINVAL, "tmjx_grad_finish: 0 .. 16 column sums, at least one without weight gradients");
+  ColsumLdGroup Q;
+  Q.n = n_sums;
+  int blocks = 0;
+  for (int i = 0; i < n_sums; i++) {
+    const tmjx_colsum_ld_problem_t &q = sums[i];
+    if (!q.partial || !q.out || q.rows < 1 || q.width < 1 || q.ld < q.width) return fail(TMJX_EINVAL, "tmjx_grad_finish: bad column-sum problem");
+    Q.p[i] = ColsumLdProblem{q.partial, q.out, q.rows, q.width, q.ld, blocks};
+    blocks += (q.width + 31) / 32;
+  }
+  hipLaunchKernelGGL(k_grad_finish, dim3(red + blocks), dim3(256), 0, (hipStream_t)stream, G, Q, red);
+  return check_launch("k_grad_finish");
 }
 
 int tmjx_rollout_store(const tmjx_rollout_store_t *q, void *stream) {
diff --git a/track_mjx_amd/hip.py b/track_mjx_amd/hip.py
--- a/track_mjx_amd/hip.py
+++ b/track_mjx_amd/hip.py
@@ -38,6 +38,10 @@
 
 class ColsumProblem(C.Structure):
     _fields_ = [("partial", C.c_void_p), ("out", C.c_void_p), ("rows", C.c_int32), ("width", C.c_int32)]
+
+
+class ColsumLdProblem(C.Structure):
+    _fields_ = [("partial", C.c_void_p), ("out", C.c_void_p), ("rows", C.c_int32), ("width", C.c_int32), ("ld", C.c_int32), ("pad_", C.c_int32)]
 
 
 class DwProblem(C.Structure):
@@ -295,6 +299,14 @@
     "tmjx_gemm_nn_ln_bwd_partial_floats": ([_i, _i], _i64),
     "tmjx_gemm_dw": ([_vp, _i, _vp, _i, _vp, _vp, _vp, _i, _i, _i, _vp], _i),
     "tmjx_gemm_dw_grouped": ([_P(DwProblem), _i, _vp], _i),
+    "tmjx_gemm_dw_slabs_grouped": ([_P(DwProblem), _i, _vp], _i),
+    "tmjx_grad_finish": ([_P(DwProblem), _i, _P(ColsumLdProblem), _i, _vp], _i),
+    "tmjx_gather_minibatch_x_ok": ([_vp, _i, _i, _i, _i], _i),
+    "tmjx_gather_minibatch_x": ([_P(Minibatch), _vp, _i, _i, _i, _vp], _i),
+    "tmjx_latent_sample_ok": ([_vp, _vp, _vp, _i, _i], _i),
+    "tmjx_latent_sample": ([_vp, _vp, _vp, _i, _i, _i, _u64, _vp, _vp], _i),
+    "tmjx_latent_sample_bwd": ([_vp] * 4 + [_i, _i, _i, _vp], _i),
+    "tmjx_latent_sample_bwd_add": ([_vp] * 5 + [_i, _i, _i, _vp], _i),
     "tmjx_gemm_dw_scratch_floats": ([_i, _i, _i], _i64),
     "tmjx_set_wrappers": ([_vp, _i, _i], _i),
     "tmjx_set_action_repeat": ([_vp, _i], _i),
```

Result: no change. 1.731 million, median of 6 (+0.5%).
